# clancylian/retinaface

Measured on NVIDIA H100. Metric: faces/sec (end-to-end detect), higher is better.
Workload: dtype f16

## Files before the change

retinaface_b200/csrc/engine.cu:

```cuda
#include <cmath>

#include "engine_internal.cuh"
#include "calibrate.cuh"
#include "preprocess.cuh"

namespace rf_eng {

std::string &create_error() {
    thread_local std::string text;
    return text;
}

void link_steps(rf_handle h) {
    auto &st = h->steps;
    for (int i = 0; i < (int)st.size(); i++) {
        st[i].deps.clear();
        for (int t : st[i].in) {
            for (int j = i - 1; j >= 0; j--) {
                bool writes = false;
                for (int o : st[j].out) writes |= (o == t);
                if (!writes) continue;
                if (st[j].lane != st[i].lane) {
                    if (std::find(st[i].deps.begin(), st[i].deps.end(), j) == st[i].deps.end()) st[i].deps.push_back(j);
                    st[j].signals = true;
                }
                break;
            }
        }
    }
    for (int l = 1; l < 3; l++) {
        h->lane_last[l] = -1;
        for (int i = 0; i < (int)st.size(); i++) if (st[i].lane == l) h->lane_last[l] = i;
        if (h->lane_last[l] >= 0) st[h->lane_last[l]].signals = true;
    }
}

void place_tensors(rf_handle h, bool keep_all) {
    auto &ts = h->tensors;
    auto &st = h->steps;
    for (int si = 0; si < (int)st.size(); si++) {
        for (int t : st[si].out) { if (ts[t].first < 0) ts[t].first = si; ts[t].last = std::max(ts[t].last, si); }
        for (int t : st[si].in) ts[t].last = std::max(ts[t].last, si);
    }
    for (int k = 0; k < (int)st.size(); k++) {
        if (st[k].lane == 0) continue;
        int join = (int)st.size() - 1;
        for (int j = k + 1; j < (int)st.size() && join == (int)st.size() - 1; j++)
            for (int d : st[j].deps)
                if (st[j].lane != st[k].lane && st[d].lane == st[k].lane && d >= k) { join = j; break; }
        for (int t : st[k].in) ts[t].last = std::max(ts[t].last, join);
        for (int t : st[k].out) ts[t].last = std::max(ts[t].last, join);
    }
    const size_t B = (size_t)h->cfg.max_batch;
    size_t top = 0;
    std::vector<int> order(ts.size());
    for (size_t i = 0; i < ts.size(); i++) order[i] = (int)i;
    std::stable_sort(order.begin(), order.end(), [&](int a, int b) { return ts[a].first < ts[b].first; });
    std::vector<int> placed;
    for (int id : order) {
        size_t sz = (ts[id].bytes_per_img * B + 255) / 256 * 256;
        size_t off = 0;
        if (keep_all) {
            off = top;
        } else {
            bool moved = true;
            while (moved) {
                moved = false;
                for (int p : placed) {
                    bool live_overlap = !(ts[p].last < ts[id].first || ts[id].last < ts[p].first);
                    size_t psz = (ts[p].bytes_per_img * B + 255) / 256 * 256;
                    bool mem_overlap = off < ts[p].offset + psz && ts[p].offset < off + sz;
                    if (live_overlap && mem_overlap) { off = ts[p].offset + psz; moved = true; }
                }
            }
        }
        ts[id].offset = off;
        top = std::max(top, off + sz);
        placed.push_back(id);
    }
    h->arena_bytes = top;
}

void make_plan(rf_handle h, bool init) {
    const rf_config &cfg = h->cfg;
    h->use_tc = cfg.precision == RF_PREC_INT8 || (cfg.precision == RF_PREC_FP16 && !(cfg.flags & RF_FLAG_NO_TENSORCORE));
    if (init && h->use_tc) CK(tc_init());
    if (cfg.precision == RF_PREC_INT8) { if (init) CK(tc_init_i8()); build_plan_i8(h); }
    else if (cfg.precision == RF_PREC_FP32) build_plan<float>(h);
    else if (h->use_tc && !(cfg.flags & RF_FLAG_LEGACY_TC)) { if (init) CK(tile_init()); build_plan_tiles(h); }
    else build_plan<__half>(h);
    link_steps(h);
    place_tensors(h, false);
}

void alloc_post_buffers(PostBuffers &pb, int anchors, int batch, int max_faces) {
    int ap2 = 1;
    while (ap2 < anchors) ap2 <<= 1;
    pb.anchors_per_image = anchors; pb.anchors_pow2 = ap2; pb.max_faces = max_faces; pb.max_batch = batch;
    const size_t B = batch;
    CK(cudaMalloc(&pb.cand_keys, sizeof(unsigned long long) * B * anchors));
    CK(cudaMalloc(&pb.cand_recs, sizeof(rf_det) * B * anchors));
    CK(cudaMalloc(&pb.cand_count, sizeof(int) * B));
    CK(cudaMemset(pb.cand_count, 0, sizeof(int) * B));
    CK(cudaMalloc(&pb.sort_scratch, sizeof(unsigned long long) * B * ap2));
    CK(cudaMalloc(&pb.flag_scratch, B * ap2));
    CK(cudaMalloc(&pb.out_dets, sizeof(rf_det) * B * max_faces));
    CK(cudaMalloc(&pb.out_counts, sizeof(int) * B));
    CK(cudaMalloc(&pb.out_total_kept, sizeof(int) * B));
    CK(cudaMemset(pb.out_counts, 0, sizeof(int) * B));
    CK(cudaMalloc(&pb.tile_done, sizeof(int) * B));
    CK(cudaMemset(pb.tile_done, 0, sizeof(int) * B));
}
void free_post_buffers(PostBuffers &pb) {
    cudaFree(pb.cand_keys); cudaFree(pb.cand_recs); cudaFree(pb.cand_count); cudaFree(pb.sort_scratch); cudaFree(pb.flag_scratch);
    cudaFree(pb.out_dets); cudaFree(pb.out_counts); cudaFree(pb.out_total_kept); cudaFree(pb.tile_done);
    pb = PostBuffers{};
}

void create_ctx(rf_handle h, Ctx &c, bool all) {
    if (all) {
        CK(cudaStreamCreateWithFlags(&c.stream, cudaStreamNonBlocking));
        for (int l = 1; l < 3; l++) CK(cudaStreamCreateWithFlags(&c.lane_stream[l], cudaStreamNonBlocking));
        c.step_event.assign(h->steps.size(), nullptr);
        for (size_t i = 0; i < h->steps.size(); i++)
            if (h->steps[i].signals) CK(cudaEventCreateWithFlags(&c.step_event[i], cudaEventDisableTiming));
        CK(cudaEventCreateWithFlags(&c.fence, cudaEventDisableTiming));
    }
    CK(cudaMalloc(&c.arena, h->arena_bytes));
    if (!all) return;
    CK(cudaMalloc(&c.d_params, sizeof(PostParams)));
    CK(cudaHostAlloc(&c.h_params, sizeof(PostParams) * Ctx::kParamSlots, cudaHostAllocDefault));
    int anchors = 0;
    for (const LevelDesc &lv : h->lv) anchors += 2 * lv.h * lv.w;
    alloc_post_buffers(c.pb, anchors, h->cfg.max_batch, h->cfg.max_faces);
}

void release_ctx(Ctx &c, bool all) {
    if (c.stream) cudaStreamSynchronize(c.stream);
    for (auto &g : c.graphs) cudaGraphExecDestroy(g.second);
    c.graphs.clear();
    cudaFree(c.arena);
    c.arena = nullptr;
    if (!all) return;
    cudaFree(c.d_params); cudaFreeHost(c.h_params);
    free_post_buffers(c.pb);
    for (auto e : c.step_event) if (e) cudaEventDestroy(e);
    for (int l = 1; l < 3; l++) if (c.lane_stream[l]) cudaStreamDestroy(c.lane_stream[l]);
    if (c.fence) cudaEventDestroy(c.fence);
    if (c.stream) cudaStreamDestroy(c.stream);
    c = Ctx{};
}

void run_steps(rf_handle h, const Run &r, bool use_lanes = true) {
    static const bool one_lane = [] { const char *e = getenv("RF_ONE_LANE"); return e && e[0] == '1'; }();
    if (one_lane) use_lanes = false;
    const Ctx &c = r.ctx;
    for (size_t i = 0; i < h->steps.size(); i++) {
        Step &st = h->steps[i];
        cudaStream_t cs = (use_lanes && st.lane) ? c.lane_stream[st.lane] : r.stream;
        if (use_lanes)
            for (int d : st.deps) CK(cudaStreamWaitEvent(cs, c.step_event[d], 0));
        st.launch(Run{c, r.n, cs, r.blobs});
        if (use_lanes && st.signals) CK(cudaEventRecord(c.step_event[i], cs));
    }
    if (use_lanes)
        for (int l = 1; l < 3; l++)
            if (h->lane_last[l] >= 0) CK(cudaStreamWaitEvent(r.stream, c.step_event[h->lane_last[l]], 0));
    if (h->comm.ready) comm_wait_in_graph(h, c, r.n, r.stream);
}

void forward_graph(rf_handle h, Ctx &c, int n) {
    if (h->cfg.flags & RF_FLAG_NO_GRAPH) {
        run_steps(h, Run{c, n, c.stream});
        CK(cudaGetLastError());
        return;
    }
    auto it = c.graphs.find(n);
    if (it == c.graphs.end()) {
        cudaGraph_t g = nullptr;
        CK(cudaStreamBeginCapture(c.stream, cudaStreamCaptureModeThreadLocal));
        run_steps(h, Run{c, n, c.stream});
        cudaError_t e = cudaStreamEndCapture(c.stream, &g);
        if (e != cudaSuccess) throw CudaFail{e, "cudaStreamEndCapture", __FILE__, __LINE__};
        cudaGraphExec_t ge = nullptr;
        e = cudaGraphInstantiate(&ge, g, 0);
        cudaGraphDestroy(g);
        if (e != cudaSuccess) throw CudaFail{e, "cudaGraphInstantiate", __FILE__, __LINE__};
        it = c.graphs.emplace(n, ge).first;
    }
    CK(cudaGraphLaunch(it->second, c.stream));
}

void set_params(rf_handle h, Ctx &c, float thr, float nms, const uint8_t *input = nullptr, unsigned comm_seq = 0) {
    PostParams *slot = c.h_params + (c.param_seq++ % Ctx::kParamSlots);
    slot->score_thr = thr;
    slot->nms_thr = nms;
    slot->input = input ? input : h->d_input;
    slot->comm_seq = comm_seq;
    slot->comm_slot = comm_seq ? comm_seq % (unsigned)h->comm.ring : 0u;
    c.cur_thr = thr;
    c.cur_nms = nms;
    CK(cudaMemcpyAsync(c.d_params, slot, sizeof(PostParams), cudaMemcpyHostToDevice, c.stream));
}

void destroy(rf_handle h) {
    if (!h) return;
    cudaSetDevice(h->device);
    for (Ctx &c : h->ctx) if (c.stream) cudaStreamSynchronize(c.stream);
    comm_release(h);
    jpeg_release(h);
    for (Ctx &c : h->ctx) release_ctx(c, true);
    free_post_buffers(h->pb_merge);
    cudaFree(h->d_weights); cudaFree(h->d_weights_h); cudaFree(h->d_weights_q); cudaFree(h->d_input); cudaFree(h->d_raw);
    for (auto p : h->d_blobs) cudaFree(p);
    h->copy_pool.reset();
    for (auto e : h->raw_ev) if (e) cudaEventDestroy(e);
    cudaFree(h->d_align_images); cudaFreeHost(h->h_align_images); cudaFree(h->d_align_crops); cudaFree(h->d_align_mats);
    cudaFreeHost(h->h_input); cudaFreeHost(h->h_raw); cudaFreeHost(h->h_dets); cudaFreeHost(h->h_counts); cudaFreeHost(h->tile_dbg);
    for (auto &sl : h->slots) {
        cudaFree(sl.d_in); cudaFreeHost(sl.h_in); cudaFreeHost(sl.h_dets); cudaFreeHost(sl.h_counts);
        if (sl.ev_h2d) cudaEventDestroy(sl.ev_h2d);
        if (sl.ev_done) cudaEventDestroy(sl.ev_done);
    }
    if (h->copy_stream) cudaStreamDestroy(h->copy_stream);
    if (h->ev0) cudaEventDestroy(h->ev0);
    if (h->ev1) cudaEventDestroy(h->ev1);
    delete h;
}

int check_n(rf_handle h, int n) {
    if (!h) return RF_ERR_INVALID_ARG;
    if (n < 0) return fail(h, RF_ERR_INVALID_ARG, "negative batch size");
    if (n > h->cfg.max_batch) return fail(h, RF_ERR_CAPACITY, fmt("batch %d exceeds max_batch %d", n, h->cfg.max_batch));
    return RF_OK;
}

}

extern "C" {

int rf_abi_version(void) { return RF_B200_ABI_VERSION; }

const char *rf_build_info(void) {
    return "librf_b200 (RetinaFace mnet25 detect path) built for sm_90a, CUDA " RF_STR(CUDART_VERSION);
}

const char *rf_status_string(int s) {
    switch (s) {
        case RF_OK: return "ok";
        case RF_ERR_INVALID_ARG: return "invalid argument";
        case RF_ERR_IO: return "i/o error";
        case RF_ERR_MODEL: return "model error";
        case RF_ERR_CUDA: return "CUDA error";
        case RF_ERR_NO_DEVICE: return "no usable CUDA device (the library has no CPU path)";
        case RF_ERR_CAPACITY: return "capacity exceeded";
        case RF_ERR_UNSUPPORTED: return "unsupported";
    }
    return "unknown status";
}

const char *rf_last_error(rf_handle h) { return h ? h->err.c_str() : create_error().c_str(); }

int rf_create(const rf_config *cfg, rf_handle *out) {
    if (out) *out = nullptr;
    if (!cfg || !out) return fail(nullptr, RF_ERR_INVALID_ARG, "rf_create: cfg and out must be non-NULL");
    if (!cfg->caffemodel_path) return fail(nullptr, RF_ERR_INVALID_ARG, "rf_create: caffemodel_path is NULL");
    rf_config cfg_local = *cfg;
    NetGraph graph;
    Model model;
    int cache_status = CACHE_NONE;
    {
        std::string err;
        int st = RF_OK;
        if (cfg->network) {
            NetworkConfig nc;
            if (!network_config(cfg->network, nc, err)) return fail(nullptr, RF_ERR_UNSUPPORTED, "rf_create: " + err);
            if (nc.ratios.size() != 1) return fail(nullptr, RF_ERR_UNSUPPORTED, fmt("rf_create: network '%s' uses %zu anchor ratios per scale; the shipped models (and this engine) have 2 anchors per position", cfg->network, nc.ratios.size()));
        }
        if (!load_model(cfg->caffemodel_path, cfg->prototxt_path ? cfg->prototxt_path : "", cfg->cache_path ? cfg->cache_path : "", model, &graph, &cache_status, err, st))
            return fail(nullptr, st, err);
        if (cfg->prototxt_path && cfg_local.net_w == 0 && cfg_local.net_h == 0) { cfg_local.net_h = graph.input_dims[2]; cfg_local.net_w = graph.input_dims[3]; }
    }
    cfg = &cfg_local;
    if (cfg->net_w <= 0 || cfg->net_h <= 0 || cfg->net_w % 32 || cfg->net_h % 32)
        return fail(nullptr, RF_ERR_INVALID_ARG, fmt("rf_create: net size %dx%d must be positive multiples of 32", cfg->net_w, cfg->net_h));
    if (cfg->max_batch <= 0 || cfg->max_batch > 4096) return fail(nullptr, RF_ERR_INVALID_ARG, "rf_create: max_batch must be in [1, 4096]");
    {
        const long long stem_elems = (long long)cfg->max_batch * (cfg->net_h / 2) * (cfg->net_w / 2) * 16;
        const long long merge_rows = (long long)cfg->max_batch * (cfg->net_h / 8);
        if (stem_elems > 0x7fffffffLL || merge_rows >= (1LL << 19) || cfg->net_w / 8 >= (1 << 12))
            return fail(nullptr, RF_ERR_CAPACITY, fmt("rf_create: max_batch %d at %dx%d exceeds the 32-bit activation index range (largest tensor: %lld elements); "
                                                      "use a smaller max_batch", cfg->max_batch, cfg->net_w, cfg->net_h, stem_elems));
    }
    if (cfg->precision != RF_PREC_FP32 && cfg->precision != RF_PREC_FP16 && cfg->precision != RF_PREC_INT8)
        return fail(nullptr, RF_ERR_INVALID_ARG, "rf_create: unknown precision");
    if (cfg->precision == RF_PREC_INT8 && !cfg->int8_table_path)
        return fail(nullptr, RF_ERR_INVALID_ARG, "rf_create: RF_PREC_INT8 needs int8_table_path (the TensorRT calibration cache of this caffemodel)");

    std::unique_ptr<rf_handle_s, void (*)(rf_handle)> H(new rf_handle_s, destroy);
    rf_handle h = H.get();
    h->cfg = *cfg;
    h->caffemodel = cfg->caffemodel_path;
    h->cfg.caffemodel_path = h->caffemodel.c_str();
    if (cfg->int8_table_path) { h->table = cfg->int8_table_path; h->cfg.int8_table_path = h->table.c_str(); }
    if (h->cfg.max_faces <= 0) h->cfg.max_faces = 256;
    if (h->cfg.max_faces > 8192) return fail(nullptr, RF_ERR_INVALID_ARG, "rf_create: max_faces must be <= 8192");
    if (h->cfg.max_image_w <= 0) h->cfg.max_image_w = h->cfg.net_w;
    if (h->cfg.max_image_h <= 0) h->cfg.max_image_h = h->cfg.net_h;
    h->cfg.max_image_w = std::max(h->cfg.max_image_w, h->cfg.net_w);
    h->cfg.max_image_h = std::max(h->cfg.max_image_h, h->cfg.net_h);
    h->device = cfg->device;
    h->elem = cfg->precision == RF_PREC_FP32 ? 4 : (cfg->precision == RF_PREC_FP16 ? 2 : 1);

    {
        std::string err;
        h->model = std::move(model);
        h->cache_status = cache_status;
        h->cfg.prototxt_path = h->cfg.cache_path = h->cfg.network = nullptr;
        if (!h->table.empty() && !read_int8_table(h->table, h->int8_scales, err)) return fail(nullptr, RF_ERR_IO, err);
    }
    int ndev = 0;
    cudaError_t e = cudaGetDeviceCount(&ndev);
    if (e != cudaSuccess || ndev == 0)
        return fail(nullptr, RF_ERR_NO_DEVICE, fmt("no CUDA device (%s); librf_b200 has no CPU path", e == cudaSuccess ? "count 0" : cudaGetErrorString(e)));
    if (cfg->device < 0 || cfg->device >= ndev) return fail(nullptr, RF_ERR_INVALID_ARG, fmt("device %d out of range (%d devices)", cfg->device, ndev));
    try {
        CK(cudaSetDevice(h->device));
        cudaDeviceProp prop;
        CK(cudaGetDeviceProperties(&prop, h->device));
        if (prop.major != 9 || prop.minor != 0)
            return fail(nullptr, RF_ERR_NO_DEVICE, fmt("device %d is sm_%d%d; librf_b200 is built for sm_90a only", h->device, prop.major, prop.minor));
        h->num_sms = prop.multiProcessorCount;
        CK(cudaEventCreate(&h->ev0));
        CK(cudaEventCreate(&h->ev1));
        CK(postproc_init());

        const int Hn = h->cfg.net_h, Wn = h->cfg.net_w, Bm = h->cfg.max_batch;
        const int strides[3] = {32, 16, 8};
        int abase = 0, pbase = 0;
        for (int l = 0; l < 3; l++) {
            LevelDesc &lv = h->lv[l];
            lv.stride = strides[l]; lv.h = Hn / strides[l]; lv.w = Wn / strides[l];
            lv.anchor_base = abase; lv.pix_base = pbase;
            base_anchors_net3(strides[l], lv.base);
            abase += 2 * lv.h * lv.w; pbase += lv.h * lv.w;
        }
        make_plan(h, true);
        CK(cudaMalloc(&h->d_weights, h->wstage.size() * sizeof(float)));
        CK(cudaMemcpy(h->d_weights, h->wstage.data(), h->wstage.size() * sizeof(float), cudaMemcpyHostToDevice));
        if (!h->wstage_h.empty()) {
            CK(cudaMalloc(&h->d_weights_h, h->wstage_h.size() * sizeof(__half)));
            CK(cudaMemcpy(h->d_weights_h, h->wstage_h.data(), h->wstage_h.size() * sizeof(__half), cudaMemcpyHostToDevice));
        }
        if (!h->wstage_q.empty()) {
            CK(cudaMalloc(&h->d_weights_q, h->wstage_q.size()));
            CK(cudaMemcpy(h->d_weights_q, h->wstage_q.data(), h->wstage_q.size(), cudaMemcpyHostToDevice));
        }
        const size_t in_bytes = (size_t)Bm * Hn * Wn * 3;
        CK(cudaMalloc(&h->d_input, in_bytes));
        CK(cudaHostAlloc(&h->h_input, in_bytes, cudaHostAllocDefault));
        h->raw_bytes = ((size_t)h->cfg.max_image_w * h->cfg.max_image_h * 3 + 255) / 256 * 256;
        h->raw_slots = (int)std::max<size_t>(1, std::min<size_t>((size_t)Bm, ((size_t)2 << 30) / h->raw_bytes));
        CK(cudaMalloc(&h->d_raw, h->raw_bytes * h->raw_slots));
        CK(cudaHostAlloc(&h->h_raw, 2 * h->raw_bytes, cudaHostAllocDefault));
        for (auto &e : h->raw_ev) CK(cudaEventCreateWithFlags(&e, cudaEventDisableTiming));
        CK(cudaHostAlloc(&h->h_dets, sizeof(rf_det) * (size_t)Bm * h->cfg.max_faces, cudaHostAllocDefault));
        CK(cudaHostAlloc(&h->h_counts, sizeof(int) * 2 * Bm, cudaHostAllocDefault));
        CK(cudaHostAlloc(&h->tile_dbg, 64, cudaHostAllocMapped));
        memset(h->tile_dbg, 0, 64);
        CK(cudaHostGetDevicePointer(&h->tile_dbg_dev, h->tile_dbg, 0));
        h->ctx.resize(h->cfg.streams <= 0 ? RF_MAX_STREAMS : std::min(h->cfg.streams, RF_MAX_STREAMS));
        for (Ctx &c : h->ctx) create_ctx(h, c, true);
        for (int l = 0; l < 3; l++) {
            const int ch[3] = {4, 8, 20};
            for (int k = 0; k < 3; k++) h->blob_elems[3 * l + k] = (size_t)ch[k] * h->lv[l].h * h->lv[l].w;
        }
        CK(cudaDeviceSynchronize());
    } catch (const CudaFail &f) {
        return fail_cuda(nullptr, f);
    } catch (const PlanFail &f) {
        return fail(nullptr, f.status, "rf_create: " + f.msg);
    }
    *out = H.release();
    return RF_OK;
}

void rf_destroy(rf_handle h) { destroy(h); }

// ... 850 lines not shown
```

retinaface_b200/csrc/engine_internal.cuh:

```cuda
#pragma once
#include <algorithm>
#include <cstdarg>
#include <cstdio>
#include <cstring>
#include <functional>
#include <map>
#include <memory>
#include <string>
#include <type_traits>
#include <vector>

#include "align.cuh"
#include "common.cuh"
#include "host_copy.h"
#include "model.h"
#include "postproc.cuh"
#include "preprocess.cuh"

using namespace rf;

#define RF_STR2(x) #x
#define RF_STR(x) RF_STR2(x)

namespace rf_eng {

constexpr int RF_NUM_SMS = 132;

struct TileChain;
std::string &create_error();

struct CudaFail { cudaError_t e; const char *what; const char *file; int line; };
struct PlanFail { int status; std::string msg; };
#define CK(call)                                                        \
    do {                                                                \
        cudaError_t _e = (call);                                        \
        if (_e != cudaSuccess) throw CudaFail{_e, #call, __FILE__, __LINE__}; \
    } while (0)

inline std::string fmt(const char *f, ...) {
    char buf[1024];
    va_list ap;
    va_start(ap, f);
    vsnprintf(buf, sizeof buf, f, ap);
    va_end(ap);
    return buf;
}

struct TensorInfo {
    std::string name;
    int h = 0, w = 0, c = 0;
    size_t bytes_per_img = 0;
    int first = -1, last = -1;
    size_t offset = 0;
};

struct Ctx {
    static constexpr int kParamSlots = 1024;
    cudaStream_t stream = nullptr, lane_stream[3] = {nullptr, nullptr, nullptr};
    std::vector<cudaEvent_t> step_event;
    unsigned char *arena = nullptr;
    PostBuffers pb{};
    PostParams *d_params = nullptr, *h_params = nullptr;
    unsigned param_seq = 0;
    float cur_thr = 0.5f, cur_nms = 0.4f;
    std::map<int, cudaGraphExec_t> graphs;
    cudaEvent_t fence = nullptr;
};

struct Run {
    const Ctx &ctx;
    int n;
    cudaStream_t stream;
    float *const *blobs = nullptr;
    bool single = false;
};

struct Step {
    std::string name;
    std::vector<int> in, out;
    std::function<void(const Run &)> launch;
    double flops_per_img = 0, bytes_per_img = 0;
    int lane = 0;
    std::vector<int> deps;
    bool signals = false;
};

}
using namespace rf_eng;

namespace rf_eng {
struct Comm {
    int rank = 0, world = 1, ring = 0;
    bool ready = false;
    unsigned char *window = nullptr;
    size_t bytes = 0;
    unsigned char *peer[RF_COMM_MAX_WORLD] = {nullptr};
    bool opened[RF_COMM_MAX_WORLD] = {false};
    unsigned seq = 0;
    unsigned *d_err = nullptr, *h_err = nullptr;
    unsigned char blob[128] = {0};
    struct Slot { rf_det *h_dets = nullptr; int *h_counts = nullptr; } slots[RF_PIPELINE_DEPTH];
};
}

struct rf_handle_s {
    rf_config cfg{};
    rf_eng::Comm comm;
    std::string caffemodel, table;
    std::string err;
    Model model;
    std::map<std::string, float> int8_scales;
    int device = 0;
    int num_sms = RF_NUM_SMS;
    int elem = 4;
    cudaEvent_t ev0 = nullptr, ev1 = nullptr;

    std::vector<TensorInfo> tensors;
    std::map<std::string, int> tensor_by_name;
    std::vector<Step> steps;
    int head_step = -1, nms_step = -1;
    std::vector<std::shared_ptr<TileChain>> chains;
    unsigned tile_mask = 0;
    int lane_last[3] = {-1, -1, -1};
    int cache_status = 0;
    int tile_expected = 0;
    std::vector<float> tile_bias_tmp;
    unsigned *tile_dbg = nullptr, *tile_dbg_dev = nullptr;
    size_t arena_bytes = 0;

    std::vector<float> wstage;
    float *d_weights = nullptr;
    std::vector<__half> wstage_h;
    __half *d_weights_h = nullptr;
    std::vector<int8_t> wstage_q;
    int8_t *d_weights_q = nullptr;
    bool use_tc = false;

    uint8_t *d_input = nullptr;
    uint8_t *h_input = nullptr;
    PostBuffers pb_merge{};
    uint8_t *d_raw = nullptr;
    uint8_t *h_raw = nullptr;
    size_t raw_bytes = 0;
    int raw_slots = 1;
    cudaEvent_t raw_ev[2] = {nullptr, nullptr};
    unsigned raw_seq = 0;
    std::unique_ptr<HostCopyPool> copy_pool;
    AlignImage *d_align_images = nullptr, *h_align_images = nullptr;
    void *d_align_crops = nullptr;
    size_t align_crops_bytes = 0;
    double *d_align_mats = nullptr;
    LevelDesc lv[3];
    HeadWeights hw[3];
    int feat_tensor[3] = {-1, -1, -1};
    float *d_blobs[9] = {nullptr};
    size_t blob_elems[9] = {0};
    rf_det *h_dets = nullptr;
    int *h_counts = nullptr;
    struct Slot {
        uint8_t *d_in = nullptr, *h_in = nullptr;
        rf_det *h_dets = nullptr;
        int *h_counts = nullptr;
        cudaEvent_t ev_h2d = nullptr, ev_done = nullptr;
        int n = 0;
        bool busy = false, gather = false;
    } slots[RF_PIPELINE_DEPTH];
    cudaStream_t copy_stream = nullptr;
    unsigned submit_seq = 0, collect_seq = 0;
    std::vector<Ctx> ctx;
    unsigned next_dev_ctx = 0;
    cudaStream_t last_stream = nullptr;
    void *jpeg = nullptr;
};

namespace rf_eng {
inline int fail(rf_handle h, int code, const std::string &msg) {
    if (h) h->err = msg; else create_error() = msg;
    return code;
}
inline int fail_cuda(rf_handle h, const CudaFail &f) {
    std::string extra;
    if (h && h->tile_dbg && h->tile_dbg[0])
        extra = fmt(" [tile chain: CTA %u timed out waiting at tile_chain.cuh:%u]", h->tile_dbg[0] >> 20, h->tile_dbg[0] & 0xfffffu);
    return fail(h, RF_ERR_CUDA, fmt("%s failed: %s (%s:%d)%s", f.what, cudaGetErrorString(f.e), f.file, f.line, extra.c_str()));
}

struct Builder {
    rf_handle h;
    int H, W;
    size_t add_weights(const std::vector<float> &v) {
        size_t off = h->wstage.size();
        h->wstage.insert(h->wstage.end(), v.begin(), v.end());
        while (h->wstage.size() % 4) h->wstage.push_back(0.f);
        return off;
    }
    size_t add_weights_h(const std::vector<__half> &v) {
        size_t off = h->wstage_h.size();
        h->wstage_h.insert(h->wstage_h.end(), v.begin(), v.end());
        while (h->wstage_h.size() % 64) h->wstage_h.push_back(__float2half(0.f));
        return off;
    }
    size_t add_weights_q(const std::vector<int8_t> &v) {
        size_t off = h->wstage_q.size();
        h->wstage_q.insert(h->wstage_q.end(), v.begin(), v.end());
        while (h->wstage_q.size() % 128) h->wstage_q.push_back(0);
        return off;
    }
    int tensor(const std::string &name, int hh, int ww, int c) {
        TensorInfo t;
        t.name = name; t.h = hh; t.w = ww; t.c = c;
        t.bytes_per_img = (size_t)hh * ww * c * h->elem;
        h->tensors.push_back(t);
        h->tensor_by_name[name] = (int)h->tensors.size() - 1;
        return (int)h->tensors.size() - 1;
    }
    void step(Step s) { h->steps.push_back(std::move(s)); }
};

constexpr int TC_SMEM_LIMIT = 200 * 1024;
struct DwGeom { int rows, nsplit, Rmax; };
template <typename T>
void build_plan(rf_handle h);
cudaError_t tc_init();
std::vector<__half> make_stem_blob(const std::vector<float> &w0, const std::vector<float> &b0, const std::vector<float> &wd,
                                   const std::vector<float> &bd, const std::vector<float> &wp, const std::vector<float> &bp);
int plan_stem_tc(Builder &B);
int plan_pair_legacy(Builder &B, int i, int tin, int ih, int iw);
void plan_conv_legacy(Builder &B, const std::string &sname, std::vector<const FoldedConv *> cs, int tin, int ih, int iw, int t0, int ld0,
                      int off0, int n0, int relu0, int t1, int ld1, int off1, int relu1, int lane = 0, int tup = -1, int up_which = 0);
int plan_fpn_merge_h2(Builder &B, const std::string &name, int tlat, int tup, int fh, int fw, int which);
template <typename T>
void plan_heads_and_nms(Builder &B, bool with_heads, bool with_nms);
std::vector<__half> pack_tc_weights(const std::vector<const FoldedConv *> &cs, std::vector<float> &bias, int &Kpad, int nsplit = 1);
void build_plan_tiles(rf_handle h);
cudaError_t tile_init();
std::string describe_chains(rf_handle h);
void comm_release(rf_handle h);
void comm_wait_in_graph(rf_handle h, const Ctx &c, int n, cudaStream_t s);
int jpeg_info(rf_handle h, const uint8_t *data, size_t len, int *w, int *hgt);
int jpeg_decode(rf_handle h, const uint8_t *const *data, const size_t *len, int n, uint8_t *const *dst, const int *w, const int *hgt, cudaStream_t s);
void jpeg_release(rf_handle h);
const char *jpeg_backend(rf_handle h);
void build_plan_i8(rf_handle h);
cudaError_t tc_init_i8();

}
```

retinaface_b200/csrc/plan_fp.cu:

```cuda
#include "engine_internal.cuh"
#include "kernels_simt.cuh"
#include "stem_tc.cuh"
#include "tc_conv.cuh"
#include "tc_dwpw2d.cuh"

namespace rf_eng {

#define CK_L(...) CK(launch_k(__VA_ARGS__))

std::vector<float> pack_gemm(const std::vector<const FoldedConv *> &cs, std::vector<float> &bias) {
    const int cin = cs[0]->cin, k = cs[0]->k;
    int N = 0;
    for (auto c : cs) N += c->cout;
    std::vector<float> w((size_t)k * k * cin * N);
    bias.assign(N, 0.f);
    int n0 = 0;
    for (auto c : cs) {
        for (int o = 0; o < c->cout; o++) {
            bias[n0 + o] = c->b[o];
            for (int ci = 0; ci < cin; ci++)
                for (int t = 0; t < k * k; t++)
                    w[((size_t)t * cin + ci) * N + n0 + o] = c->w[((size_t)o * cin + ci) * k * k + t];
        }
        n0 += c->cout;
    }
    return w;
}

template <typename T>
void launch_gemm(const T *in, int ldin, int cin, const float *wk, const float *bias, int N, int ks, OutSplit<T> outs,
                 int n, int H, int W, cudaStream_t s) {
    long M = (long)n * H * W;
    int bn = (N % 64 == 0) ? 64 : (N % 32 == 0 ? 32 : 16);
    dim3 grid((unsigned)((M + 63) / 64), (N + bn - 1) / bn);
#define RF_GEMM(BN_, KS_) CK_L(k_conv_gemm<T, BN_, KS_>, grid, dim3(256), 0, s, in, ldin, cin, wk, bias, N, outs, n, H, W)
    if (ks == 1) { if (bn == 64) RF_GEMM(64, 1); else if (bn == 32) RF_GEMM(32, 1); else RF_GEMM(16, 1); }
    else { if (bn == 64) RF_GEMM(64, 3); else if (bn == 32) RF_GEMM(32, 3); else RF_GEMM(16, 3); }
#undef RF_GEMM
}

std::vector<__half> pack_tc_weights(const std::vector<const FoldedConv *> &cs, std::vector<float> &bias, int &Kpad, int nsplit) {
    const int cin = cs[0]->cin, k = cs[0]->k;
    int N = 0;
    for (auto c : cs) N += c->cout;
    const int K = k * k * cin;
    Kpad = (K + 15) / 16 * 16;
    const int Ns = N / nsplit;
    std::vector<__half> img((size_t)Kpad * N, __float2half(0.f));
    bias.assign(N, 0.f);
    int n0 = 0;
    for (auto c : cs) {
        for (int o = 0; o < c->cout; o++) {
            const int n = n0 + o, sl = n / Ns, nl = n % Ns;
            bias[n] = c->b[o];
            for (int ci = 0; ci < cin; ci++)
                for (int t = 0; t < k * k; t++) {
                    const int kk = t * cin + ci;
                    img[(size_t)sl * Kpad * Ns + ((size_t)(kk / 8) * Ns + nl) * 8 + (kk % 8)] =
                        __float2half(c->w[((size_t)o * cin + ci) * k * k + t]);
                }
        }
        n0 += c->cout;
    }
    return img;
}

void launch_tc_conv(const TcConvArgs &a_in, cudaStream_t s) {
    TcConvArgs a = a_in;
    a.mul_Wp = fast_div_mul((uint32_t)a.Wp); a.mul_Hp = fast_div_mul((uint32_t)a.Hp); a.mul_H = fast_div_mul((uint32_t)a.H);
    const long P = (long)a.nimg * a.Hp * a.Wp;
    const unsigned grid = (unsigned)((P + 127) / 128);
    const size_t smem = tc_conv_smem_bytes(a);
    switch (tc_n_bucket(a.N)) {
        case 32: if (a.up) CK_L(k_tc_conv_staged<32, true>, dim3(grid), dim3(TC_THREADS), smem, s, a); else CK_L(k_tc_conv_staged<32, false>, dim3(grid), dim3(TC_THREADS), smem, s, a); break;
        case 64: if (a.up) CK_L(k_tc_conv_staged<64, true>, dim3(grid), dim3(TC_THREADS), smem, s, a); else CK_L(k_tc_conv_staged<64, false>, dim3(grid), dim3(TC_THREADS), smem, s, a); break;
        case 128: if (a.up) CK_L(k_tc_conv_staged<128, true>, dim3(grid), dim3(TC_THREADS), smem, s, a); else CK_L(k_tc_conv_staged<128, false>, dim3(grid), dim3(TC_THREADS), smem, s, a); break;
        default: if (a.up) CK_L(k_tc_conv_staged<256, true>, dim3(grid), dim3(TC_THREADS), smem, s, a); else CK_L(k_tc_conv_staged<256, false>, dim3(grid), dim3(TC_THREADS), smem, s, a); break;
    }
}
void launch_tc_dwpw(const TcDwArgs &a_in, int nsplit, cudaStream_t s) {
    TcDwArgs a = a_in;
    a.mul_Wp = fast_div_mul((uint32_t)a.Wp); a.mul_Hp = fast_div_mul((uint32_t)a.Hp);
    a.mul_OW = fast_div_mul((uint32_t)a.OW); a.mul_OH = fast_div_mul((uint32_t)a.OH);
    const long M = (long)a.nimg * a.OH * a.OW;
    dim3 grid((unsigned)((M + a.rows - 1) / a.rows), nsplit);
    const size_t smem = tc_dw_smem_bytes(a);
    switch (tc_n_bucket(a.N)) {
        case 32: CK_L(k_tc_dwpw_staged<32>, grid, dim3(TC_THREADS), smem, s, a); break;
        case 64: CK_L(k_tc_dwpw_staged<64>, grid, dim3(TC_THREADS), smem, s, a); break;
        case 128: CK_L(k_tc_dwpw_staged<128>, grid, dim3(TC_THREADS), smem, s, a); break;
        default: CK_L(k_tc_dwpw_staged<256>, grid, dim3(TC_THREADS), smem, s, a); break;
    }
}
void launch_tc_dwpw_2d(const TcDw2dArgs &a, cudaStream_t s) {
    const dim3 grid((unsigned)(a.tiles_x * a.tiles_y * a.nimg));
    const size_t smem = tc_dw2d_smem_bytes(a);
    switch (tc_n_bucket(a.N)) {
        case 32: CK_L(k_tc_dwpw_2d<32>, grid, dim3(TC_THREADS), smem, s, a); break;
        case 64: CK_L(k_tc_dwpw_2d<64>, grid, dim3(TC_THREADS), smem, s, a); break;
        case 128: CK_L(k_tc_dwpw_2d<128>, grid, dim3(TC_THREADS), smem, s, a); break;
        default: CK_L(k_tc_dwpw_2d<256>, grid, dim3(TC_THREADS), smem, s, a); break;
    }
}

cudaError_t tc_init() {
    cudaError_t e;
#define RF_TC_ATTR(K_) if ((e = cudaFuncSetAttribute(K_, cudaFuncAttributeMaxDynamicSharedMemorySize, TC_SMEM_LIMIT))) return e
    RF_TC_ATTR((k_tc_conv_staged<32, false>)); RF_TC_ATTR((k_tc_conv_staged<64, false>)); RF_TC_ATTR((k_tc_conv_staged<128, false>)); RF_TC_ATTR((k_tc_conv_staged<256, false>));
    RF_TC_ATTR((k_tc_conv_staged<32, true>)); RF_TC_ATTR((k_tc_conv_staged<64, true>)); RF_TC_ATTR((k_tc_conv_staged<128, true>)); RF_TC_ATTR((k_tc_conv_staged<256, true>));
    RF_TC_ATTR(k_tc_dwpw_staged<32>); RF_TC_ATTR(k_tc_dwpw_staged<64>); RF_TC_ATTR(k_tc_dwpw_staged<128>); RF_TC_ATTR(k_tc_dwpw_staged<256>);
    RF_TC_ATTR(k_tc_dwpw_2d<32>); RF_TC_ATTR(k_tc_dwpw_2d<64>); RF_TC_ATTR(k_tc_dwpw_2d<128>); RF_TC_ATTR(k_tc_dwpw_2d<256>);
#undef RF_TC_ATTR
    return cudaSuccess;
}

DwGeom dw_geometry(int C, int N, int IH, int IW, int S) {
    const int OH = IH / S, OW = IW / S, Wp = IW + 2, Hp = IH + 1, Kpad = (C + 15) / 16 * 16;
    auto centre = [&](long m) { long ox = m % OW, oy = (m / OW) % OH, b = m / ((long)OW * OH); return (b * Hp + oy * S) * Wp + ox * S + 1; };
    for (int rows : {128, 64}) {
        if (rows == 128 && OH * OW <= 28 * 28) continue;
        for (int nsplit : {1, 2, 4}) {
            if ((N / nsplit) % 16) continue;
            long g = rows, t = (long)OH * OW;
            while (t) { long u = g % t; g = t; t = u; }
            const long M = ((long)rows / g + 1) * OH * OW;
            int R = 0;
            for (long m0 = 0; m0 < M; m0 += rows) {
                long ml = std::min(m0 + rows, M) - 1;
                R = std::max(R, (int)(centre(ml) - centre(m0) + 2 * (Wp + 1) + 1));
            }
            R |= 1;
            TcDwArgs a{};
            a.C = C; a.Rmax = R; a.Kpad = Kpad; a.N = N / nsplit; a.rows = rows;
            if (R <= TC_MAX_R && tc_dw_smem_bytes(a) <= (size_t)TC_SMEM_LIMIT) return {rows, nsplit, R};
        }
    }
    return {0, 0, 0};
}

std::vector<__half> make_stem_blob(const std::vector<float> &w0, const std::vector<float> &b0, const std::vector<float> &wd,
                                          const std::vector<float> &bd, const std::vector<float> &wp, const std::vector<float> &bp) {
    std::vector<__half> b0img(2 * 4 * 16 * 8, __float2half(0.f)), b1img(2 * 16 * 8, __float2half(0.f));
    for (int k = 0; k < 27; k++)
        for (int o = 0; o < 8; o++) {
            const float wv = w0[k * 8 + o];
            const __half hi = __float2half(wv);
            b0img[((k / 8) * 16 + o) * 8 + (k % 8)] = hi;
            b0img[((4 + k / 8) * 16 + o) * 8 + (k % 8)] = __float2half(wv - __half2float(hi));
        }
    for (int c = 0; c < 8; c++)
        for (int o = 0; o < 16; o++) b1img[(0 * 16 + o) * 8 + c] = __float2half(wp[c * 16 + o]);
    std::vector<__half> blob(STEM_CONST_BYTES / 2, __float2half(0.f));
    memcpy(blob.data(), b0img.data(), STEM_B0_BYTES);
    memcpy(reinterpret_cast<unsigned char *>(blob.data()) + STEM_B0_BYTES, b1img.data(), STEM_B1_BYTES);
    std::vector<float> fl;
    fl.insert(fl.end(), b0.begin(), b0.begin() + 8);
    fl.insert(fl.end(), wd.begin(), wd.begin() + 72);
    fl.insert(fl.end(), bd.begin(), bd.begin() + 8);
    fl.insert(fl.end(), bp.begin(), bp.begin() + 16);
    fl.insert(fl.end(), wp.begin(), wp.begin() + 128);
    memcpy(reinterpret_cast<unsigned char *>(blob.data()) + STEM_B0_BYTES + STEM_B1_BYTES, fl.data(), STEM_F_FLOATS * 4);
    return blob;
}


int plan_pair_legacy(Builder &B, int i, int tin, int ih, int iw) {
    rf_handle h = B.h;
    const Model &m = h->model;
    auto T_ = [h](const Run &r, int id) { return reinterpret_cast<__half *>(r.ctx.arena + h->tensors[id].offset); };
    auto Wd = [h](size_t off) { return h->d_weights + off; };
    const double es = h->elem;
    const FoldedConv &dw = m.conv("mobilenet0_conv" + std::to_string(i) + "_fwd");
    const FoldedConv &pw = m.conv("mobilenet0_conv" + std::to_string(i + 1) + "_fwd");
    const int C = dw.cout, S = dw.stride;
    std::vector<float> wd(9 * C);
    for (int c = 0; c < C; c++)
        for (int t = 0; t < 9; t++) wd[t * C + c] = dw.w[(size_t)c * 9 + t];
    size_t owd = B.add_weights(wd), obd = B.add_weights(dw.b);
    const int oh = ih / S, ow_ = iw / S;
    const int N = pw.cout;
    const DwGeom geo = dw_geometry(C, N, ih, iw, S);
    if (geo.rows == 0) throw PlanFail{RF_ERR_UNSUPPORTED, fmt("layer mobilenet0_conv%d (%dx%d, %d channels) does not fit shared memory", i, iw, ih, C)};
    std::vector<float> bias;
    int Kpad = 0;
    std::vector<__half> img = pack_tc_weights({&pw}, bias, Kpad, geo.nsplit);
    size_t oimg = B.add_weights_h(img), obp = B.add_weights(bias);
    int tpw = B.tensor("mobilenet0_relu" + std::to_string(i + 1) + "_fwd", oh, ow_, N);
    Step s;
    s.name = fmt("tc_dw%d+pw%d_s%d_%dto%d", i, i + 1, S, C, N);
    s.in = {tin}; s.out = {tpw};
    s.flops_per_img = 2.0 * oh * ow_ * C * 9 + 2.0 * oh * ow_ * C * N;
    s.bytes_per_img = ((double)ih * iw * C + (double)oh * ow_ * N) * es;
    const bool tiles2d = oh * ow_ > 56 * 56 && C >= 16 && C <= 64 && geo.nsplit == 1 && !(h->cfg.flags & RF_FLAG_DW_1D);
    if (tiles2d) s.name = fmt("tc2d_dw%d+pw%d_s%d_%dto%d", i, i + 1, S, C, N);
    s.launch = [=](const Run &r) {
        if (tiles2d) {
            TcDw2dArgs a{};
            a.in = T_(r, tin); a.C = C; a.nimg = r.n; a.IH = ih; a.IW = iw; a.OH = oh; a.OW = ow_; a.S = S; a.N = N;
            a.TH = 8;
            const int t16 = (ow_ + 15) / 16, t14 = (ow_ + 13) / 14;
            a.TW = t14 < t16 ? 14 : 16;
            tc_dw2d_finish(a);
            a.wimg = h->d_weights_h + oimg; a.bias = Wd(obp); a.dw_w = Wd(owd); a.dw_b = Wd(obd); a.out = T_(r, tpw);
            launch_tc_dwpw_2d(a, r.stream);
            return;
        }
        TcDwArgs a{};
        a.in = T_(r, tin); a.C = C; a.nimg = r.n; a.IH = ih; a.IW = iw; a.OH = oh; a.OW = ow_; a.S = S;
        a.N = N / geo.nsplit; a.Ntotal = N; a.Kpad = Kpad; a.rows = geo.rows; a.Wp = iw + 2; a.Hp = ih + 1; a.Rmax = geo.Rmax;
        a.wimg = h->d_weights_h + oimg; a.bias = Wd(obp); a.dw_w = Wd(owd); a.dw_b = Wd(obd); a.out = T_(r, tpw);
        launch_tc_dwpw(a, geo.nsplit, r.stream);
    };
    B.step(std::move(s));
    return tpw;
}

void plan_conv_legacy(Builder &B, const std::string &sname, std::vector<const FoldedConv *> cs, int tin, int ih, int iw, int t0, int ld0,
                      int off0, int n0, int relu0, int t1, int ld1, int off1, int relu1, int lane, int tup, int up_which) {
    rf_handle h = B.h;
    const Model &m = h->model;
    auto T_ = [h](const Run &r, int id) { return reinterpret_cast<__half *>(r.ctx.arena + h->tensors[id].offset); };
    auto Wd = [h](size_t off) { return h->d_weights + off; };
    const double es = h->elem;
    std::vector<float> bias;
    int Kpad = 0;
    std::vector<__half> img = pack_tc_weights(cs, bias, Kpad);
    size_t oimg = B.add_weights_h(img), ob = B.add_weights(bias);
    const int N = (int)bias.size(), cin = cs[0]->cin, ks = cs[0]->k;
    size_t oup = tup >= 0 ? B.add_weights(m.up_w[up_which]) : 0;
    if (cin & (cin - 1)) throw PlanFail{RF_ERR_UNSUPPORTED, fmt("convolution %s: %d input channels (the tensor-core kernels index by shifts: powers of two only)", sname.c_str(), cin)};
    TcConvArgs probe{};
    probe.Cin = cin; probe.taps = ks * ks; probe.N = N; probe.R = (ks == 3 ? 128 + 2 * (iw + 3) : 128) | 1;
    if (tup >= 0) { probe.up = reinterpret_cast<const __half *>(1); probe.Cmax = (((probe.R / (iw + 2) + 2) / 2 + 3) * (iw / 2)) | 1; }
    if (tc_conv_smem_bytes(probe) > (size_t)TC_SMEM_LIMIT || probe.R > TC_MAX_R)
        throw PlanFail{RF_ERR_UNSUPPORTED, fmt("convolution %s (%dx%d map) does not fit shared memory", sname.c_str(), iw, ih)};
    Step s;
    s.name = "tc_" + sname;
    s.lane = lane;
    s.in = {tin};
    if (tup >= 0) s.in.push_back(tup);
    s.out = {t0};
    if (t1 >= 0) s.out.push_back(t1);
    s.flops_per_img = 2.0 * ih * iw * cin * ks * ks * N + (tup >= 0 ? 2.0 * ih * iw * cin * 4 : 0.0);
    s.bytes_per_img = ((double)ih * iw * cin + (double)ih * iw * N + (tup >= 0 ? (double)(ih / 2) * (iw / 2) * cin : 0.0)) * es;
    s.launch = [=](const Run &r) {
        TcConvArgs a{};
        a.in = T_(r, tin); a.Cin = cin; a.nimg = r.n; a.H = ih; a.W = iw; a.taps = ks * ks; a.N = N;
        a.Wp = ks == 3 ? iw + 2 : iw; a.Hp = ks == 3 ? ih + 1 : ih;
        a.R = (ks == 3 ? 128 + 2 * (iw + 3) : 128) | 1;
        a.wimg = h->d_weights_h + oimg; a.bias = Wd(ob);
        a.out = TcOut{T_(r, t0) + off0, ld0, n0, relu0, t1 >= 0 ? T_(r, t1) + off1 : nullptr, ld1, relu1};
        if (tup >= 0) { a.up = T_(r, tup); a.up_w = Wd(oup); a.Cmax = (((a.R / a.Wp + 2) / 2 + 3) * (iw / 2)) | 1; }
        launch_tc_conv(a, r.stream);
    };
    B.step(std::move(s));
}

int plan_fpn_merge_h2(Builder &B, const std::string &name, int tlat, int tup, int fh, int fw, int which) {
    rf_handle h = B.h;
    const Model &m = h->model;
    auto T_ = [h](const Run &r, int id) { return reinterpret_cast<__half *>(r.ctx.arena + h->tensors[id].offset); };
    const double es = h->elem;
    std::vector<__half> uwh(16 * 64);
    for (int c = 0; c < 64; c++)
        for (int t = 0; t < 16; t++) uwh[t * 64 + c] = __float2half(m.up_w[which][c * 16 + t]);
    size_t ouw = B.add_weights_h(uwh);
    int plus = B.tensor(name, fh, fw, 64);
    Step s;
    s.name = "fpn_merge" + name + "_upsample+add_h2";
    s.in = {tlat, tup}; s.out = {plus};
    s.flops_per_img = 2.0 * fh * fw * 64 * 4;
    s.bytes_per_img = ((double)fh * fw * 64 * 2 + (double)(fh / 2) * (fw / 2) * 64) * es;
    s.launch = [=](const Run &r) {
        CK(launch_k(k_fpn_merge_h2, dim3((unsigned)((fw * 8 + 127) / 128), (unsigned)fh, (unsigned)r.n), dim3(128), 0, r.stream, (const __half *)T_(r, tlat), (const __half *)T_(r, tup),
                    (__half *)T_(r, plus), (const __half *)(h->d_weights_h + ouw), r.n, fh, fw, 64));
    };
    B.step(std::move(s));
    return plus;
}

template <typename T>
void plan_heads_and_nms(Builder &B, bool with_heads, bool with_nms) {
    rf_handle h = B.h;
    const Model &m = h->model;
    auto T_ = [h](const Run &r, int id) { return reinterpret_cast<T *>(r.ctx.arena + h->tensors[id].offset); };
    auto Wd = [h](size_t off) { return h->d_weights + off; };
    const double es = h->elem;
    const int H = h->cfg.net_h, W = h->cfg.net_w;
    const int h32 = H / 32, w32 = W / 32, h16 = H / 16, w16 = W / 16, h8 = H / 8, w8 = W / 8;
    if (with_heads) {
        size_t hw_off[3], hb_off[3];
        const int strides[3] = {32, 16, 8};
        for (int l = 0; l < 3; l++) {
            std::string st = "_stride" + std::to_string(strides[l]);
            const FoldedConv *cs[3] = {&m.conv("face_rpn_cls_score" + st), &m.conv("face_rpn_bbox_pred" + st),
                                       &m.conv("face_rpn_landmark_pred" + st)};
            std::vector<float> w(32 * 64), b(32);
            int r = 0;
            for (auto c : cs)
                for (int o = 0; o < c->cout; o++, r++) {
                    b[r] = c->b[o];
                    for (int ci = 0; ci < 64; ci++) w[r * 64 + ci] = c->w[(size_t)o * 64 + ci];
                }
            hw_off[l] = B.add_weights(w);
            hb_off[l] = B.add_weights(b);
        }
        Step s;
        s.name = "heads_1x1+softmax+decode_all_levels";
        s.in = {h->feat_tensor[0], h->feat_tensor[1], h->feat_tensor[2]};
        double px = (double)h32 * w32 + (double)h16 * w16 + (double)h8 * w8;
        s.flops_per_img = 2.0 * px * 64 * 4;
        s.bytes_per_img = px * 64 * es;
        int f0 = h->feat_tensor[0], f1 = h->feat_tensor[1], f2 = h->feat_tensor[2];
        size_t w0 = hw_off[0], w1 = hw_off[1], w2 = hw_off[2], b0 = hb_off[0], b1 = hb_off[1], b2 = hb_off[2];
        s.launch = [=](const Run &r) {
            const T *feat[3] = {T_(r, f0), T_(r, f1), T_(r, f2)};
            HeadWeights hws[3] = {{Wd(w0), Wd(b0), 1.f}, {Wd(w1), Wd(b1), 1.f}, {Wd(w2), Wd(b2), 1.f}};
            launch_head_decode<T>(feat, hws, h->lv, r.n, W, H, r.ctx.d_params, r.ctx.pb, r.blobs, r.stream, with_nms);
        };
        if (with_nms) s.name = "heads_1x1+softmax+decode+nms_all_levels";
        h->head_step = (int)h->steps.size();
        B.step(std::move(s));
        if (with_nms) return;
    }
    if (with_nms) {
        Step s;
        s.name = "sort+nms";
        s.in = {h->feat_tensor[0], h->feat_tensor[1], h->feat_tensor[2]};
        s.flops_per_img = 0;
        s.bytes_per_img = 0;
        s.launch = [=](const Run &r) { launch_nms(r.n, r.ctx.d_params, r.ctx.pb, r.stream); };
        h->nms_step = (int)h->steps.size();
        B.step(std::move(s));
    }
}
template void plan_heads_and_nms<float>(Builder &, bool, bool);
template void plan_heads_and_nms<__half>(Builder &, bool, bool);

int plan_stem_tc(Builder &B) {
    rf_handle h = B.h;
    const Model &m = h->model;
    const int H = h->cfg.net_h, W = h->cfg.net_w;
    auto T_ = [h](const Run &r, int id) { return reinterpret_cast<__half *>(r.ctx.arena + h->tensors[id].offset); };
    auto Wd = [h](size_t off) { return h->d_weights + off; };
    const double es = h->elem;
    const int cur_h = H / 2, cur_w = W / 2;
    const FoldedConv &c0 = m.conv("mobilenet0_conv0_fwd"), &dw = m.conv("mobilenet0_conv1_fwd"), &pw = m.conv("mobilenet0_conv2_fwd");
    std::vector<float> w0(27 * 8), wd(72), wp(128);
    for (int o = 0; o < 8; o++)
        for (int cb = 0; cb < 3; cb++)
            for (int t = 0; t < 9; t++) w0[(t * 3 + cb) * 8 + o] = c0.w[((size_t)o * 3 + (2 - cb)) * 9 + t];
    for (int c = 0; c < 8; c++)
        for (int t = 0; t < 9; t++) wd[t * 8 + c] = dw.w[(size_t)c * 9 + t];
    for (int o = 0; o < 16; o++)
        for (int c = 0; c < 8; c++) wp[c * 16 + o] = pw.w[(size_t)o * 8 + c];
    size_t ow0 = B.add_weights(w0), ob0 = B.add_weights(c0.b), owd = B.add_weights(wd), obd = B.add_weights(dw.b),
           owp = B.add_weights(wp), obp = B.add_weights(pw.b);
    std::vector<__half> blob = make_stem_blob(w0, c0.b, wd, dw.b, wp, pw.b);
    size_t oblob = B.add_weights_h(blob);
    const bool simt_stem = (h->cfg.flags & (RF_FLAG_SIMT_STEM | RF_FLAG_NO_TENSORCORE)) != 0;
    int out = B.tensor("mobilenet0_relu2_fwd", cur_h, cur_w, 16);
    Step s;
    s.name = simt_stem ? "stem_conv0+dw1+pw2_u8_to_16ch" : "tc_stem_conv0+dw1+pw2_u8_to_16ch";
    s.out = {out};
    s.flops_per_img = 2.0 * cur_h * cur_w * (8 * 27 + 8 * 9 + 8 * 16);
    s.bytes_per_img = (double)H * W * 3 + (double)cur_h * cur_w * 16 * es;
    s.launch = [=](const Run &r) {
        const int tiles = ((H / 2 + 15) / 16) * ((W / 2 + 15) / 16);
        if (simt_stem) {
            StemWeights sw{Wd(ow0), Wd(ob0), Wd(owd), Wd(obd), Wd(owp), Wd(obp)};
            CK(launch_k(k_stem<__half>, dim3((unsigned)(tiles * r.n)), dim3(256), 0, r.stream, (const PostParams *)r.ctx.d_params, (__half *)T_(r, out), sw, r.n, H, W, 1.0f));
        } else {
            StemTcArgs a{reinterpret_cast<const unsigned char *>(h->d_weights_h + oblob)};
            CK(launch_k(k_stem_tc<__half>, dim3((unsigned)((W / 2 + 15) / 16), (unsigned)((H / 2 + 15) / 16), (unsigned)r.n), dim3(256), 0, r.stream, (const PostParams *)r.ctx.d_params, (__half *)T_(r, out), a, r.n, H, W, 1.0f));
        }
    };
    B.step(std::move(s));
    return out;
}

template <typename T>
void build_plan(rf_handle h) {
    Builder B{h, h->cfg.net_h, h->cfg.net_w};
    const Model &m = h->model;
    const int H = h->cfg.net_h, W = h->cfg.net_w;
    auto T_ = [h](const Run &r, int id) { return reinterpret_cast<T *>(r.ctx.arena + h->tensors[id].offset); };
    auto Wd = [h](size_t off) { return h->d_weights + off; };
    const double es = h->elem;

    int first_pair = 1;
    int cur_h = H / 2, cur_w = W / 2, cur_c = 8;
    int cur = -1;
    bool stem_done = false;
    if constexpr (std::is_same<T, __half>::value) {
        if (h->use_tc) {
            cur = plan_stem_tc(B);
            cur_c = 16;
            first_pair = 3;
            stem_done = true;
        }
    }
    if (!stem_done) {
    cur = B.tensor("mobilenet0_relu0_fwd", cur_h, cur_w, 8);
    {
        const FoldedConv &c = m.conv("mobilenet0_conv0_fwd");
        std::vector<float> wk(27 * 8);
        for (int o = 0; o < 8; o++)
            for (int cb = 0; cb < 3; cb++)
                for (int t = 0; t < 9; t++) wk[(t * 3 + cb) * 8 + o] = c.w[((size_t)o * 3 + (2 - cb)) * 9 + t];
        size_t ow = B.add_weights(wk), ob = B.add_weights(c.b);
        int out = cur;
        Step s;
        s.name = "conv0_u8_3x3s2_bn_relu";
        s.out = {out};
        s.flops_per_img = 2.0 * cur_h * cur_w * 8 * 27;
        s.bytes_per_img = (double)H * W * 3 + (double)cur_h * cur_w * 8 * es;
        s.launch = [=](const Run &r) {
            long total = (long)r.n * (H / 2) * (W / 2);
            CK_L(k_conv0<T>, dim3((unsigned)((total + 255) / 256)), dim3(256), 0, r.stream, (const PostParams *)r.ctx.d_params, T_(r, out), Wd(ow), Wd(ob), r.n, H, W);
        };
        B.step(std::move(s));
    }
    }
    int c1 = -1, c2 = -1, c3 = -1;
    for (int i = first_pair; i <= 26; i += 2) {
        const FoldedConv &dw = m.conv("mobilenet0_conv" + std::to_string(i) + "_fwd");
        const FoldedConv &pw = m.conv("mobilenet0_conv" + std::to_string(i + 1) + "_fwd");
        const int C = dw.cout, S = dw.stride;
        std::vector<float> wd(9 * C);
        for (int c = 0; c < C; c++)
            for (int t = 0; t < 9; t++) wd[t * C + c] = dw.w[(size_t)c * 9 + t];
        size_t owd = B.add_weights(wd), obd = B.add_weights(dw.b);
        const int ih = cur_h, iw = cur_w, oh = cur_h / S, ow_ = cur_w / S;
        int tin = cur;
        if constexpr (std::is_same<T, __half>::value) {
            if (h->use_tc) {
                cur = plan_pair_legacy(B, i, tin, ih, iw);
                cur_h = oh; cur_w = ow_; cur_c = pw.cout;
                if (i + 1 == 10) c1 = cur;
                if (i + 1 == 22) c2 = cur;
                if (i + 1 == 26) c3 = cur;
                continue;
            }
        }
        int tdw = B.tensor("mobilenet0_relu" + std::to_string(i) + "_fwd", oh, ow_, C);
        {
            Step s;
            s.name = fmt("dw%d_3x3s%d_c%d", i, S, C);
            s.in = {tin}; s.out = {tdw};
            s.flops_per_img = 2.0 * oh * ow_ * C * 9;
            s.bytes_per_img = ((double)ih * iw * C + (double)oh * ow_ * C) * es;
            s.launch = [=](const Run &r) {
                long total = (long)r.n * oh * ow_ * (C / 8);
                unsigned g = (unsigned)((total + 255) / 256);
                if (S == 1) CK_L(k_dw3x3<T, 1>, dim3(g), dim3(256), 0, r.stream, (const T *)T_(r, tin), T_(r, tdw), Wd(owd), Wd(obd), r.n, ih, iw, C);
                else CK_L(k_dw3x3<T, 2>, dim3(g), dim3(256), 0, r.stream, (const T *)T_(r, tin), T_(r, tdw), Wd(owd), Wd(obd), r.n, ih, iw, C);
            };
            B.step(std::move(s));
        }
        std::vector<float> bias;
        std::vector<float> wk = pack_gemm({&pw}, bias);
        size_t owp = B.add_weights(wk), obp = B.add_weights(bias);
        const int N = pw.cout;
        int tpw = B.tensor("mobilenet0_relu" + std::to_string(i + 1) + "_fwd", oh, ow_, N);
        {
            Step s;
            s.name = fmt("pw%d_1x1_%dto%d", i + 1, C, N);
            s.in = {tdw}; s.out = {tpw};
            s.flops_per_img = 2.0 * oh * ow_ * C * N;
            s.bytes_per_img = ((double)oh * ow_ * C + (double)oh * ow_ * N) * es;
            s.launch = [=](const Run &r) {
                OutSplit<T> o{T_(r, tpw), N, N, 1, nullptr, 0, 0};
                launch_gemm<T>(T_(r, tdw), C, C, Wd(owp), Wd(obp), N, 1, o, r.n, oh, ow_, r.stream);
            };
            B.step(std::move(s));
        }
        cur = tpw; cur_h = oh; cur_w = ow_; cur_c = N;
        if (i + 1 == 10) c1 = cur;
        if (i + 1 == 22) c2 = cur;
        if (i + 1 == 26) c3 = cur;
    }
    (void)cur_c;

    auto conv_step = [&](const std::string &sname, std::vector<const FoldedConv *> cs, int tin, int ih, int iw,
                         int t0, int ld0, int off0, int n0, int relu0, int t1, int ld1, int off1, int relu1, int lane = 0,
                         int tup = -1, int up_which = 0) {
        if constexpr (std::is_same<T, __half>::value) {
            if (h->use_tc) {
                plan_conv_legacy(B, sname, cs, tin, ih, iw, t0, ld0, off0, n0, relu0, t1, ld1, off1, relu1, lane, tup, up_which);
                return;
            }
        }
        std::vector<float> bias;
        std::vector<float> wk = pack_gemm(cs, bias);
        size_t ow = B.add_weights(wk), ob = B.add_weights(bias);
        const int N = (int)bias.size(), cin = cs[0]->cin, ks = cs[0]->k;
        const int ldin = h->tensors[tin].c;
        Step s;
        s.name = sname;
        s.lane = lane;
        s.in = {tin};
        s.out = {t0};
        if (t1 >= 0) s.out.push_back(t1);
        s.flops_per_img = 2.0 * ih * iw * cin * ks * ks * N;
        s.bytes_per_img = ((double)ih * iw * cin + (double)ih * iw * N) * es;
        s.launch = [=](const Run &r) {
            OutSplit<T> o{T_(r, t0) + off0, ld0, n0, relu0, t1 >= 0 ? T_(r, t1) + off1 : nullptr, ld1, relu1};
            launch_gemm<T>(T_(r, tin), ldin, cin, Wd(ow), Wd(ob), N, ks, o, r.n, ih, iw, r.stream);
        };
        B.step(std::move(s));
    };
    auto ssh = [&](const std::string &lvname, int tin, int fh, int fw, int level, int lane) {
        const std::string p = "rf_" + lvname + "_det";
        int cat = B.tensor(p + "_concat_relu", fh, fw, 64);
        int ctx1 = B.tensor(p + "_context_conv1_relu", fh, fw, 16);
        int ctx31 = B.tensor(p + "_context_conv3_1_relu", fh, fw, 16);
        conv_step("ssh_" + lvname + "_conv1+ctx1_3x3_64to48", {&m.conv(p + "_conv1"), &m.conv(p + "_context_conv1")}, tin, fh,
                  fw, cat, 64, 0, 32, 1, ctx1, 16, 0, 1, lane);
        conv_step("ssh_" + lvname + "_ctx2+ctx3_1_3x3_16to32", {&m.conv(p + "_context_conv2"), &m.conv(p + "_context_conv3_1")},
                  ctx1, fh, fw, cat, 64, 32, 16, 1, ctx31, 16, 0, 1, lane);
        conv_step("ssh_" + lvname + "_ctx3_2_3x3_16to16", {&m.conv(p + "_context_conv3_2")}, ctx31, fh, fw, cat, 64, 48, 16, 1,
                  -1, 0, 0, 0, lane);
        h->feat_tensor[level] = cat;
    };
    auto upadd = [&](const std::string &name, int tlat, int tup, int fh, int fw, int which) {
        size_t ow = B.add_weights(m.up_w[which]);
        int out = B.tensor(name, fh, fw, 64);
        Step s;
        s.name = "upsample_add" + name;
        s.in = {tlat, tup}; s.out = {out};
        s.flops_per_img = 2.0 * fh * fw * 64 * 4;
        s.bytes_per_img = ((double)fh * fw * 64 * 2 + (double)(fh / 2) * (fw / 2) * 64) * es;
        s.launch = [=](const Run &r) {
            long total = (long)r.n * fh * fw * 8;
            CK_L(k_upsample_add<T>, dim3((unsigned)((total + 255) / 256)), dim3(256), 0, r.stream, (const T *)T_(r, tlat), (const T *)T_(r, tup), T_(r, out), Wd(ow), r.n,
                     fh, fw, 64, fh / 2, fw / 2);
        };
        B.step(std::move(s));
        return out;
    };
    const int h32 = H / 32, w32 = W / 32, h16 = H / 16, w16 = W / 16, h8 = H / 8, w8 = W / 8;
    const bool lanes = h->use_tc;
    auto move_last_step_after_producer = [&](int tensor_id) {
        int pos = 0;
        for (int i = (int)h->steps.size() - 2; i >= 0 && !pos; i--)
            for (int t : h->steps[i].out) if (t == tensor_id) { pos = i + 1; break; }
        Step st = std::move(h->steps.back());
        h->steps.pop_back();
        h->steps.insert(h->steps.begin() + pos, std::move(st));
    };
    int lat3 = B.tensor("rf_c3_lateral_relu", h32, w32, 64);
    int lat2 = B.tensor("rf_c2_lateral_relu", h16, w16, 64);
    int lat1 = B.tensor("rf_c1_red_conv_relu", h8, w8, 64);
    conv_step("c1_red_1x1_64to64", {&m.conv("rf_c1_red_conv")}, c1, h8, w8, lat1, 64, 0, 64, 1, -1, 0, 0, 0, lanes ? 1 : 0);
    if (lanes) move_last_step_after_producer(c1);
    conv_step("c2_lateral_1x1_128to64", {&m.conv("rf_c2_lateral")}, c2, h16, w16, lat2, 64, 0, 64, 1, -1, 0, 0, 0, lanes ? 2 : 0);
    if (lanes) move_last_step_after_producer(c2);
    conv_step("c3_lateral_1x1_256to64", {&m.conv("rf_c3_lateral")}, c3, h32, w32, lat3, 64, 0, 64, 1, -1, 0, 0, 0);
    ssh("c3", lat3, h32, w32, 0, lanes ? 1 : 0);
    int aggr2 = B.tensor("rf_c2_aggr_relu", h16, w16, 64);
    if (h->use_tc) {
        conv_step("c2_upsample+add+aggr_3x3_64to64", {&m.conv("rf_c2_aggr")}, lat2, h16, w16, aggr2, 64, 0, 64, 1, -1, 0, 0, 0, 0, lat3, 0);
    } else {
        int plus0 = upadd("_plus0", lat2, lat3, h16, w16, 0);
        conv_step("c2_aggr_3x3_64to64", {&m.conv("rf_c2_aggr")}, plus0, h16, w16, aggr2, 64, 0, 64, 1, -1, 0, 0, 0);
    }
    ssh("c2", aggr2, h16, w16, 1, lanes ? 2 : 0);
    int aggr1 = B.tensor("rf_c1_aggr_relu", h8, w8, 64);
    const long c1_tiles = ((long)h->cfg.max_batch * (h8 + 1) * (w8 + 2) + 127) / 128;
    if (h->use_tc && c1_tiles <= h->num_sms) {
        conv_step("c1_upsample+add+aggr_3x3_64to64", {&m.conv("rf_c1_aggr")}, lat1, h8, w8, aggr1, 64, 0, 64, 1, -1, 0, 0, 0, 0, aggr2, 1);
    } else if (h->use_tc) {
        if constexpr (std::is_same<T, __half>::value) {
            int plus1 = plan_fpn_merge_h2(B, "_plus1", lat1, aggr2, h8, w8, 1);
            conv_step("c1_aggr_3x3_64to64", {&m.conv("rf_c1_aggr")}, plus1, h8, w8, aggr1, 64, 0, 64, 1, -1, 0, 0, 0);
        }
    } else {
        int plus1 = upadd("_plus1", lat1, aggr2, h8, w8, 1);
        conv_step("c1_aggr_3x3_64to64", {&m.conv("rf_c1_aggr")}, plus1, h8, w8, aggr1, 64, 0, 64, 1, -1, 0, 0, 0);
    }
    ssh("c1", aggr1, h8, w8, 2, 0);

    plan_heads_and_nms<T>(B, true, true);
}

template void build_plan<float>(rf_handle h);
template void build_plan<__half>(rf_handle h);

}
```

retinaface_b200/csrc/plan_i8.cu:

```cuda
#include "engine_internal.cuh"
#include "kernels_simt.cuh"
#include "stem_tc.cuh"
#include "tc_conv_i8.cuh"
#include "tc_dwpw2d_i8.cuh"

namespace rf_eng {

struct QWeights { std::vector<int8_t> img; std::vector<float> mult, bq; };

QWeights pack_tc_weights_i8(const std::vector<const FoldedConv *> &cs, float s_in, const std::vector<float> &s_out, int groups, int nsplit) {
    const int cin = cs[0]->cin, k = cs[0]->k, taps = k * k;
    int N = 0;
    for (auto c : cs) N += c->cout;
    const int Ns = N / nsplit;
    QWeights q;
    q.img.assign((size_t)taps * groups * 16 * N, 0);
    q.mult.resize(N); q.bq.resize(N);
    int n0 = 0;
    for (auto c : cs) {
        const size_t per = (size_t)cin * taps;
        for (int o = 0; o < c->cout; o++) {
            const int n = n0 + o, sl = n / Ns, nl = n % Ns;
            float mx = 0.f;
            for (size_t i = 0; i < per; i++) mx = std::max(mx, std::fabs(c->w[o * per + i]));
            const float sw = mx > 0.f ? mx / 127.0f : 1.0f;
            q.mult[n] = (float)((double)s_in * (double)sw / (double)s_out[n]);
            q.bq[n] = (float)((double)c->b[o] / (double)s_out[n]);
            for (int ci = 0; ci < cin; ci++)
                for (int t = 0; t < taps; t++) {
                    double v = std::nearbyint((double)c->w[((size_t)o * cin + ci) * taps + t] / (double)sw);
                    v = std::max(-127.0, std::min(127.0, v));
                    const int g = t * groups + ci / 16;
                    q.img[(size_t)sl * taps * groups * 16 * Ns + ((size_t)g * Ns + nl) * 16 + (ci % 16)] = (int8_t)v;
                }
        }
        n0 += c->cout;
    }
    return q;
}

void launch_tc_conv_i8(const TcConvArgsI8 &a_in, cudaStream_t s) {
    TcConvArgsI8 a = a_in;
    a.mul_Wp = fast_div_mul((uint32_t)a.Wp); a.mul_Hp = fast_div_mul((uint32_t)a.Hp); a.mul_H = fast_div_mul((uint32_t)a.H);
    const long P = (long)a.nimg * a.Hp * a.Wp;
    const dim3 grid((unsigned)((P + 127) / 128));
    const size_t smem = tc_conv_i8_smem_bytes(a);
#define RF_I8C(NT_) if (a.up) launch_k(k_tc_conv_staged_i8<NT_, true>, grid, dim3(TC_THREADS), smem, s, a); else launch_k(k_tc_conv_staged_i8<NT_, false>, grid, dim3(TC_THREADS), smem, s, a)
    switch (tc_n_bucket(a.N)) {
        case 32: RF_I8C(32); break;
        case 64: RF_I8C(64); break;
        case 128: RF_I8C(128); break;
        default: RF_I8C(256); break;
    }
#undef RF_I8C
}
void launch_tc_dwpw_2d_i8(const TcDw2dArgsI8 &a, cudaStream_t s) {
    const dim3 grid((unsigned)a.tiles_x, (unsigned)a.tiles_y, (unsigned)a.nimg);
    const size_t smem = tc_dw2d_i8_smem_bytes(a);
    switch (tc_n_bucket(a.N)) {
        case 32: launch_k(k_tc_dwpw_2d_i8<32>, grid, dim3(TC_THREADS), smem, s, a); break;
        case 64: launch_k(k_tc_dwpw_2d_i8<64>, grid, dim3(TC_THREADS), smem, s, a); break;
        case 128: launch_k(k_tc_dwpw_2d_i8<128>, grid, dim3(TC_THREADS), smem, s, a); break;
        default: launch_k(k_tc_dwpw_2d_i8<256>, grid, dim3(TC_THREADS), smem, s, a); break;
    }
}

void launch_tc_dwpw_i8(const TcDwArgsI8 &a_in, int nsplit, cudaStream_t s) {
    TcDwArgsI8 a = a_in;
    a.mul_Wp = fast_div_mul((uint32_t)a.Wp); a.mul_Hp = fast_div_mul((uint32_t)a.Hp);
    a.mul_OW = fast_div_mul((uint32_t)a.OW); a.mul_OH = fast_div_mul((uint32_t)a.OH);
    const long M = (long)a.nimg * a.OH * a.OW;
    const dim3 grid((unsigned)((M + a.rows - 1) / a.rows), nsplit);
    const size_t smem = tc_dw_i8_smem_bytes(a);
    switch (tc_n_bucket(a.N)) {
        case 32: if (a.C >= 64) launch_k(k_tc_dwpw_staged_i8<32, true>, grid, dim3(TC_THREADS), smem, s, a); else launch_k(k_tc_dwpw_staged_i8<32, false>, grid, dim3(TC_THREADS), smem, s, a); break;
        case 64: if (a.C >= 64) launch_k(k_tc_dwpw_staged_i8<64, true>, grid, dim3(TC_THREADS), smem, s, a); else launch_k(k_tc_dwpw_staged_i8<64, false>, grid, dim3(TC_THREADS), smem, s, a); break;
        case 128: if (a.C >= 64) launch_k(k_tc_dwpw_staged_i8<128, true>, grid, dim3(TC_THREADS), smem, s, a); else launch_k(k_tc_dwpw_staged_i8<128, false>, grid, dim3(TC_THREADS), smem, s, a); break;
        default: if (a.C >= 64) launch_k(k_tc_dwpw_staged_i8<256, true>, grid, dim3(TC_THREADS), smem, s, a); else launch_k(k_tc_dwpw_staged_i8<256, false>, grid, dim3(TC_THREADS), smem, s, a); break;
    }
}
cudaError_t tc_init_i8() {
    cudaError_t e;
#define RF_TC_ATTR(K_) if ((e = cudaFuncSetAttribute(K_, cudaFuncAttributeMaxDynamicSharedMemorySize, TC_SMEM_LIMIT))) return e
    RF_TC_ATTR((k_tc_conv_staged_i8<32, false>)); RF_TC_ATTR((k_tc_conv_staged_i8<64, false>)); RF_TC_ATTR((k_tc_conv_staged_i8<128, false>)); RF_TC_ATTR((k_tc_conv_staged_i8<256, false>));
    RF_TC_ATTR((k_tc_conv_staged_i8<32, true>)); RF_TC_ATTR((k_tc_conv_staged_i8<64, true>)); RF_TC_ATTR((k_tc_conv_staged_i8<128, true>)); RF_TC_ATTR((k_tc_conv_staged_i8<256, true>));
    RF_TC_ATTR((k_tc_dwpw_staged_i8<32, true>)); RF_TC_ATTR((k_tc_dwpw_staged_i8<64, true>)); RF_TC_ATTR((k_tc_dwpw_staged_i8<128, true>)); RF_TC_ATTR((k_tc_dwpw_staged_i8<256, true>));
    RF_TC_ATTR((k_tc_dwpw_staged_i8<32, false>)); RF_TC_ATTR((k_tc_dwpw_staged_i8<64, false>)); RF_TC_ATTR((k_tc_dwpw_staged_i8<128, false>)); RF_TC_ATTR((k_tc_dwpw_staged_i8<256, false>));
    RF_TC_ATTR(k_tc_dwpw_2d_i8<32>); RF_TC_ATTR(k_tc_dwpw_2d_i8<64>); RF_TC_ATTR(k_tc_dwpw_2d_i8<128>); RF_TC_ATTR(k_tc_dwpw_2d_i8<256>);
#undef RF_TC_ATTR
    return cudaSuccess;
}

DwGeom dw_geometry_i8(int C, int N, int IH, int IW, int S) {
    const int OH = IH / S, OW = IW / S, Wp = IW + 2, Hp = IH + 1, Kpad = (C + 31) / 32 * 32;
    auto centre = [&](long m) { long ox = m % OW, oy = (m / OW) % OH, b = m / ((long)OW * OH); return (b * Hp + oy * S) * Wp + ox * S + 1; };
    for (int rows : {128, 64}) {
        if (rows == 128 && OH * OW <= 28 * 28) continue;
        for (int nsplit : {1, 2, 4}) {
            if ((N / nsplit) % 16) continue;
            long g = rows, t = (long)OH * OW;
            while (t) { long u = g % t; g = t; t = u; }
            const long M = ((long)rows / g + 1) * OH * OW;
            int R = 0;
            for (long m0 = 0; m0 < M; m0 += rows) {
                long ml = std::min(m0 + rows, M) - 1;
                R = std::max(R, (int)(centre(ml) - centre(m0) + 2 * (Wp + 1) + 1));
            }
            R |= 1;
            TcDwArgsI8 a{};
            a.C = C; a.Rmax = R; a.Kpad = Kpad; a.N = N / nsplit; a.rows = rows;
            if (R <= TC_MAX_R && tc_dw_i8_smem_bytes(a) <= (size_t)TC_SMEM_LIMIT) return {rows, nsplit, R};
        }
    }
    return {0, 0, 0};
}

void build_plan_i8(rf_handle h) {
    Builder B{h, h->cfg.net_h, h->cfg.net_w};
    const Model &m = h->model;
    const int H = h->cfg.net_h, W = h->cfg.net_w;
    auto Q_ = [h](const Run &r, int id) { return reinterpret_cast<int8_t *>(r.ctx.arena + h->tensors[id].offset); };
    auto Wd = [h](size_t off) { return h->d_weights + off; };
    auto scale_of = [h](const std::string &name) -> float {
        auto it = h->int8_scales.find(name);
        if (it == h->int8_scales.end()) throw PlanFail{RF_ERR_MODEL, "INT8 calibration table lacks the scale of tensor '" + name + "'"};
        return it->second;
    };
    auto tscale = [&](int id) { return scale_of(h->tensors[id].name); };

    int cur_h = H / 2, cur_w = W / 2;
    int cur = B.tensor("mobilenet0_relu2_fwd", cur_h, cur_w, 16);
    {
        const FoldedConv &c0 = m.conv("mobilenet0_conv0_fwd"), &dw = m.conv("mobilenet0_conv1_fwd"), &pw = m.conv("mobilenet0_conv2_fwd");
        std::vector<float> w0(27 * 8), wd(72), wp(128);
        for (int o = 0; o < 8; o++)
            for (int cb = 0; cb < 3; cb++)
                for (int t = 0; t < 9; t++) w0[(t * 3 + cb) * 8 + o] = c0.w[((size_t)o * 3 + (2 - cb)) * 9 + t];
        for (int c = 0; c < 8; c++)
            for (int t = 0; t < 9; t++) wd[t * 8 + c] = dw.w[(size_t)c * 9 + t];
        for (int o = 0; o < 16; o++)
            for (int c = 0; c < 8; c++) wp[c * 16 + o] = pw.w[(size_t)o * 8 + c];
        size_t ow0 = B.add_weights(w0), ob0 = B.add_weights(c0.b), owd = B.add_weights(wd), obd = B.add_weights(dw.b),
               owp = B.add_weights(wp), obp = B.add_weights(pw.b);
        const float inv = 1.0f / tscale(cur);
        int out = cur;
        Step s;
        s.name = "stem_conv0+dw1+pw2_u8_to_16ch_i8";
        s.out = {out};
        s.flops_per_img = 2.0 * cur_h * cur_w * (8 * 27 + 8 * 9 + 8 * 16);
        s.bytes_per_img = (double)H * W * 3 + (double)cur_h * cur_w * 16;
        const bool simt_stem = (h->cfg.flags & (RF_FLAG_SIMT_STEM | RF_FLAG_NO_TENSORCORE)) != 0;
        size_t oblob = B.add_weights_h(make_stem_blob(w0, c0.b, wd, dw.b, wp, pw.b));
        if (!simt_stem) s.name = "tc_stem_conv0+dw1+pw2_u8_to_16ch_i8";
        s.launch = [=](const Run &r) {
            if (simt_stem) {
                StemWeights sw{Wd(ow0), Wd(ob0), Wd(owd), Wd(obd), Wd(owp), Wd(obp)};
                const int tiles = ((H / 2 + 15) / 16) * ((W / 2 + 15) / 16);
                launch_k(k_stem<int8_t>, dim3((unsigned)(tiles * r.n)), dim3(256), 0, r.stream, (const PostParams *)r.ctx.d_params, Q_(r, out), sw, r.n, H, W, inv);
            } else {
                StemTcArgs a{reinterpret_cast<const unsigned char *>(h->d_weights_h + oblob)};
                launch_k(k_stem_tc<int8_t>, dim3((unsigned)((W / 2 + 15) / 16), (unsigned)((H / 2 + 15) / 16), (unsigned)r.n), dim3(256), 0, r.stream,
                         (const PostParams *)r.ctx.d_params, Q_(r, out), a, r.n, H, W, inv);
            }
        };
        B.step(std::move(s));
    }
    int c1 = -1, c2 = -1, c3 = -1;
    for (int i = 3; i <= 26; i += 2) {
        const FoldedConv &dw = m.conv("mobilenet0_conv" + std::to_string(i) + "_fwd");
        const FoldedConv &pw = m.conv("mobilenet0_conv" + std::to_string(i + 1) + "_fwd");
        const int C = dw.cout, S = dw.stride, N = pw.cout;
        const int ih = cur_h, iw = cur_w, oh = cur_h / S, ow_ = cur_w / S;
        const float s_in = tscale(cur), s_mid = scale_of("mobilenet0_relu" + std::to_string(i) + "_fwd");
        std::vector<float> wd(9 * C);
        for (int c = 0; c < C; c++)
            for (int t = 0; t < 9; t++) wd[t * C + c] = dw.w[(size_t)c * 9 + t] * s_in;
        size_t owd = B.add_weights(wd), obd = B.add_weights(dw.b);
        const DwGeom geo = dw_geometry_i8(C, N, ih, iw, S);
        if (geo.rows == 0) throw PlanFail{RF_ERR_UNSUPPORTED, fmt("INT8 layer mobilenet0_conv%d (%dx%d, %d channels) does not fit shared memory", i, iw, ih, C)};
        int tin = cur;
        int tpw = B.tensor("mobilenet0_relu" + std::to_string(i + 1) + "_fwd", oh, ow_, N);
        const int Kpad = (C + 31) / 32 * 32;
        std::vector<float> s_out(N, tscale(tpw));
        QWeights q = pack_tc_weights_i8({&pw}, s_mid, s_out, Kpad / 16, geo.nsplit);
        size_t oimg = B.add_weights_q(q.img), omul = B.add_weights(q.mult), obq = B.add_weights(q.bq);
        const float inv_mid = 1.0f / s_mid;
        Step s;
        s.name = fmt("i8_dw%d+pw%d_s%d_%dto%d", i, i + 1, S, C, N);
        s.in = {tin}; s.out = {tpw};
        s.flops_per_img = 2.0 * oh * ow_ * C * 9 + 2.0 * oh * ow_ * C * N;
        s.bytes_per_img = (double)ih * iw * C + (double)oh * ow_ * N;
        const bool tiles2d = oh * ow_ > 56 * 56 && C >= 16 && C <= 64 && geo.nsplit == 1 && !(h->cfg.flags & RF_FLAG_DW_1D);
        if (tiles2d) s.name = fmt("i8_2d_dw%d+pw%d_s%d_%dto%d", i, i + 1, S, C, N);
        s.launch = [=](const Run &r) {
            if (tiles2d) {
                TcDw2dArgsI8 a{};
                a.in = Q_(r, tin); a.C = C; a.nimg = r.n; a.IH = ih; a.IW = iw; a.OH = oh; a.OW = ow_; a.S = S; a.N = N; a.Kpad = Kpad;
                a.TH = 8;
                a.TW = (ow_ + 13) / 14 < (ow_ + 15) / 16 ? 14 : 16;
                tc_dw2d_i8_finish(a);
                a.wimg = h->d_weights_q + oimg; a.mult = Wd(omul); a.bq = Wd(obq); a.dw_w = Wd(owd); a.dw_b = Wd(obd); a.inv_mid = inv_mid;
                a.out = Q_(r, tpw);
                launch_tc_dwpw_2d_i8(a, r.stream);
                return;
            }
            TcDwArgsI8 a{};
            a.in = Q_(r, tin); a.C = C; a.nimg = r.n; a.IH = ih; a.IW = iw; a.OH = oh; a.OW = ow_; a.S = S;
            a.N = N / geo.nsplit; a.Ntotal = N; a.Kpad = Kpad; a.rows = geo.rows; a.Wp = iw + 2; a.Hp = ih + 1; a.Rmax = geo.Rmax;
            a.wimg = h->d_weights_q + oimg; a.mult = Wd(omul); a.bq = Wd(obq); a.dw_w = Wd(owd); a.dw_b = Wd(obd); a.inv_mid = inv_mid;
            a.out = Q_(r, tpw);
            launch_tc_dwpw_i8(a, geo.nsplit, r.stream);
        };
        B.step(std::move(s));
        cur = tpw; cur_h = oh; cur_w = ow_;
        if (i + 1 == 10) c1 = cur;
        if (i + 1 == 22) c2 = cur;
        if (i + 1 == 26) c3 = cur;
    }
    auto conv_step = [&](const std::string &sname, std::vector<const FoldedConv *> cs, int tin, int ih, int iw, int t0, int ld0, int off0,
                         int n0, int relu0, int t1, int ld1, int off1, int relu1, int lane, int tup, int up_which, int tlat_for_up) {
        (void)tlat_for_up;
        const int cin = cs[0]->cin, ks = cs[0]->k;
        int N = 0;
        for (auto c : cs) N += c->cout;
        std::vector<float> s_out(N);
        for (int n = 0; n < N; n++) s_out[n] = n < n0 ? tscale(t0) : tscale(t1);
        const float s_in = tup >= 0 ? scale_of(up_which == 0 ? "_plus0" : "_plus1") : tscale(tin);
        QWeights q = pack_tc_weights_i8(cs, s_in, s_out, tc_i8_gs(cin), 1);
        size_t oimg = B.add_weights_q(q.img), omul = B.add_weights(q.mult), obq = B.add_weights(q.bq);
        size_t oup = 0;
        float lat_mul = 0.f;
        if (tup >= 0) {
            std::vector<float> wq(16 * cin);
            const float s_up = tscale(tup);
            for (int c = 0; c < cin; c++)
                for (int t = 0; t < 16; t++) wq[t * cin + c] = (float)((double)m.up_w[up_which][c * 16 + t] * (double)s_up / (double)s_in);
            oup = B.add_weights(wq);
            lat_mul = (float)((double)tscale(tin) / (double)s_in);
        }
        Step s;
        s.name = "i8_" + sname;
        s.lane = lane;
        s.in = {tin};
        if (tup >= 0) s.in.push_back(tup);
        s.out = {t0};
        if (t1 >= 0) s.out.push_back(t1);
        s.flops_per_img = 2.0 * ih * iw * cin * ks * ks * N;
        s.bytes_per_img = (double)ih * iw * cin + (double)ih * iw * N + (tup >= 0 ? (double)(ih / 2) * (iw / 2) * cin : 0.0);
        s.launch = [=](const Run &r) {
            TcConvArgsI8 a{};
            a.in = Q_(r, tin); a.Cin = cin; a.nimg = r.n; a.H = ih; a.W = iw; a.taps = ks * ks; a.N = N;
            a.Wp = ks == 3 ? iw + 2 : iw; a.Hp = ks == 3 ? ih + 1 : ih;
            a.R = (ks == 3 ? 128 + 2 * (iw + 3) : 128) | 1;
            a.wimg = h->d_weights_q + oimg; a.mult = Wd(omul); a.bq = Wd(obq);
            a.out = TcOutI8{Q_(r, t0) + off0, ld0, n0, relu0, t1 >= 0 ? Q_(r, t1) + off1 : nullptr, ld1, relu1};
            if (tup >= 0) { a.up = Q_(r, tup); a.up_wq = Wd(oup); a.lat_mul = lat_mul; a.Cmax = (((a.R / a.Wp + 2) / 2 + 3) * (iw / 2)) | 1; }
            launch_tc_conv_i8(a, r.stream);
        };
        B.step(std::move(s));
    };
    auto move_last_step_after_producer = [&](int tensor_id) {
        int pos = 0;
        for (int i = (int)h->steps.size() - 2; i >= 0 && !pos; i--)
            for (int t : h->steps[i].out) if (t == tensor_id) { pos = i + 1; break; }
        Step st = std::move(h->steps.back());
        h->steps.pop_back();
        h->steps.insert(h->steps.begin() + pos, std::move(st));
    };
    auto ssh = [&](const std::string &lvname, int tin, int fh, int fw, int level, int lane) {
        const std::string p = "rf_" + lvname + "_det";
        int cat = B.tensor(p + "_concat_relu", fh, fw, 64);
        int ctx1 = B.tensor(p + "_context_conv1_relu", fh, fw, 16);
        int ctx31 = B.tensor(p + "_context_conv3_1_relu", fh, fw, 16);
        conv_step("ssh_" + lvname + "_conv1+ctx1_3x3_64to48", {&m.conv(p + "_conv1"), &m.conv(p + "_context_conv1")}, tin, fh, fw, cat, 64, 0, 32, 1,
                  ctx1, 16, 0, 1, lane, -1, 0, -1);
        conv_step("ssh_" + lvname + "_ctx2+ctx3_1_3x3_16to32", {&m.conv(p + "_context_conv2"), &m.conv(p + "_context_conv3_1")}, ctx1, fh, fw, cat,
                  64, 32, 16, 1, ctx31, 16, 0, 1, lane, -1, 0, -1);
        conv_step("ssh_" + lvname + "_ctx3_2_3x3_16to16", {&m.conv(p + "_context_conv3_2")}, ctx31, fh, fw, cat, 64, 48, 16, 1, -1, 0, 0, 0, lane, -1,
                  0, -1);
        h->feat_tensor[level] = cat;
    };
    const int h32 = H / 32, w32 = W / 32, h16 = H / 16, w16 = W / 16, h8 = H / 8, w8 = W / 8;
    int lat3 = B.tensor("rf_c3_lateral_relu", h32, w32, 64);
    int lat2 = B.tensor("rf_c2_lateral_relu", h16, w16, 64);
    int lat1 = B.tensor("rf_c1_red_conv_relu", h8, w8, 64);
    conv_step("c1_red_1x1_64to64", {&m.conv("rf_c1_red_conv")}, c1, h8, w8, lat1, 64, 0, 64, 1, -1, 0, 0, 0, 1, -1, 0, -1);
    move_last_step_after_producer(c1);
    conv_step("c2_lateral_1x1_128to64", {&m.conv("rf_c2_lateral")}, c2, h16, w16, lat2, 64, 0, 64, 1, -1, 0, 0, 0, 2, -1, 0, -1);
    move_last_step_after_producer(c2);
    conv_step("c3_lateral_1x1_256to64", {&m.conv("rf_c3_lateral")}, c3, h32, w32, lat3, 64, 0, 64, 1, -1, 0, 0, 0, 0, -1, 0, -1);
    ssh("c3", lat3, h32, w32, 0, 1);
    int aggr2 = B.tensor("rf_c2_aggr_relu", h16, w16, 64);
    conv_step("c2_upsample+add+aggr_3x3_64to64", {&m.conv("rf_c2_aggr")}, lat2, h16, w16, aggr2, 64, 0, 64, 1, -1, 0, 0, 0, 0, lat3, 0, lat2);
    ssh("c2", aggr2, h16, w16, 1, 2);
    int aggr1 = B.tensor("rf_c1_aggr_relu", h8, w8, 64);
    const long c1_tiles = ((long)h->cfg.max_batch * (h8 + 1) * (w8 + 2) + 127) / 128;
    if (c1_tiles <= h->num_sms) {
        conv_step("c1_upsample+add+aggr_3x3_64to64", {&m.conv("rf_c1_aggr")}, lat1, h8, w8, aggr1, 64, 0, 64, 1, -1, 0, 0, 0, 0, aggr2, 1, lat1);
    } else {
        int plus1 = B.tensor("_plus1", h8, w8, 64);
        const float s_out = tscale(plus1), s_up = tscale(aggr2), s_lat = tscale(lat1);
        std::vector<float> wq(16 * 64);
        for (int c = 0; c < 64; c++)
            for (int t = 0; t < 16; t++) wq[t * 64 + c] = (float)((double)m.up_w[1][c * 16 + t] * (double)s_up / (double)s_out);
        size_t owq = B.add_weights(wq);
        const float lat_mul = (float)((double)s_lat / (double)s_out);
        Step s;
        s.name = "i8_fpn_merge_c1_upsample+add";
        s.in = {lat1, aggr2}; s.out = {plus1};
        s.flops_per_img = 2.0 * h8 * w8 * 64 * 4;
        s.bytes_per_img = (double)h8 * w8 * 64 * 2 + (double)(h8 / 2) * (w8 / 2) * 64;
        s.launch = [=](const Run &r) {
            launch_k(k_fpn_merge_i8, dim3((unsigned)((w8 * 4 + 127) / 128), (unsigned)h8, (unsigned)r.n), dim3(128), 0, r.stream, (const int8_t *)Q_(r, lat1), (const int8_t *)Q_(r, aggr2), Q_(r, plus1),
                     Wd(owq), lat_mul, r.n, h8, w8, 64);
        };
        B.step(std::move(s));
        conv_step("c1_aggr_3x3_64to64", {&m.conv("rf_c1_aggr")}, plus1, h8, w8, aggr1, 64, 0, 64, 1, -1, 0, 0, 0, 0, -1, 0, -1);
    }
    ssh("c1", aggr1, h8, w8, 2, 0);
    size_t hw_off[3], hb_off[3];
    float hs[3];
    const int strides[3] = {32, 16, 8};
    for (int l = 0; l < 3; l++) {
        std::string st = "_stride" + std::to_string(strides[l]);
        const FoldedConv *cs[3] = {&m.conv("face_rpn_cls_score" + st), &m.conv("face_rpn_bbox_pred" + st), &m.conv("face_rpn_landmark_pred" + st)};
        std::vector<float> w(32 * 64), b(32);
        int r = 0;
        for (auto c : cs)
            for (int o = 0; o < c->cout; o++, r++) {
                b[r] = c->b[o];
                for (int ci = 0; ci < 64; ci++) w[r * 64 + ci] = c->w[(size_t)o * 64 + ci];
            }
        hw_off[l] = B.add_weights(w);
        hb_off[l] = B.add_weights(b);
        hs[l] = tscale(h->feat_tensor[l]);
    }
    {
        Step s;
        s.name = "i8_heads_1x1+softmax+decode_all_levels";
        s.in = {h->feat_tensor[0], h->feat_tensor[1], h->feat_tensor[2]};
        double px = (double)h32 * w32 + (double)h16 * w16 + (double)h8 * w8;
        s.flops_per_img = 2.0 * px * 64 * 4;
        s.bytes_per_img = px * 64;
        int f0 = h->feat_tensor[0], f1 = h->feat_tensor[1], f2 = h->feat_tensor[2];
        size_t w0 = hw_off[0], w1 = hw_off[1], w2 = hw_off[2], b0 = hb_off[0], b1 = hb_off[1], b2 = hb_off[2];
        float s0 = hs[0], s1 = hs[1], s2 = hs[2];
        s.launch = [=](const Run &r) {
            const int8_t *feat[3] = {Q_(r, f0), Q_(r, f1), Q_(r, f2)};
            HeadWeights hws[3] = {{Wd(w0), Wd(b0), s0}, {Wd(w1), Wd(b1), s1}, {Wd(w2), Wd(b2), s2}};
            launch_head_decode<int8_t>(feat, hws, h->lv, r.n, W, H, r.ctx.d_params, r.ctx.pb, r.blobs, r.stream, true);
        };
        s.name = "i8_heads_1x1+softmax+decode+nms_all_levels";
        h->head_step = (int)h->steps.size();
        B.step(std::move(s));
    }
}

}
```

retinaface_b200/csrc/stem_tc.cuh:

```cuda
#pragma once
#include "tc_conv.cuh"

namespace rf {

constexpr int STEM_B0_BYTES = 2 * 4 * 16 * 8 * 2, STEM_B1_BYTES = 2 * 16 * 8 * 2, STEM_F_FLOATS = 8 + 72 + 8 + 16 + 128;
constexpr int STEM_CONST_BYTES = STEM_B0_BYTES + STEM_B1_BYTES + STEM_F_FLOATS * 4;
static_assert(STEM_CONST_BYTES % 16 == 0, "bulk copy size");
struct StemTcArgs {
    const unsigned char *consts;
};

constexpr int STEM_LBO0 = 384 * 16 + 16;
constexpr int STEM_LBO1 = 256 * 16 + 16;

template <typename OutT>
__global__ void __launch_bounds__(256, 4) k_stem_tc(const PostParams *__restrict__ run, OutT *__restrict__ out, StemTcArgs w,
                                                    int n, int H, int W, float out_inv_scale) {
    constexpr bool I8 = sizeof(OutT) == 1;
    __shared__ __align__(16) uint8_t s_in[37][116];
    __shared__ __align__(128) unsigned char s_a0[4 * STEM_LBO0];
    __shared__ __align__(128) unsigned char s_const[STEM_CONST_BYTES];
    __shared__ __align__(8) uint64_t bar_w;

    unsigned char *s_a1 = s_a0;
    constexpr int STEM_C0_OFF = (2 * STEM_LBO1 + 127) / 128 * 128;
    static_assert(STEM_C0_OFF + 18 * 18 * 8 * 4 <= 4 * STEM_LBO0, "conv0 ring must fit behind the pointwise operand");
    float (*s_c0)[18 * 18][4] = reinterpret_cast<float (*)[18 * 18][4]>(s_a0 + STEM_C0_OFF);
    const int tid = threadIdx.x, warp = tid >> 5, lane = tid & 31;
    const int OH = H >> 1, OW = W >> 1;
    const int b = blockIdx.z;
    const int oy0 = blockIdx.y << 4, ox0 = blockIdx.x << 4;

    const __half *s_b0 = reinterpret_cast<const __half *>(s_const), *s_b1 = reinterpret_cast<const __half *>(s_const + STEM_B0_BYTES);
    const float *s_bias0 = reinterpret_cast<const float *>(s_const + STEM_B0_BYTES + STEM_B1_BYTES);
    const float *s_wd = s_bias0 + 8, *s_bias2 = s_bias0 + 8 + 72 + 8;
    if (tid == 0) {
        tc::mbar_init(&bar_w, 1);
        asm volatile("fence.mbarrier_init.release.cluster;" ::: "memory");
        tc::mbar_expect_tx(&bar_w, STEM_CONST_BYTES);
        tc::bulk_g2s(s_const, w.consts, STEM_CONST_BYTES, &bar_w);
    }
    pdl_trigger();
    pdl_wait();
    const uint8_t *__restrict__ img = run->input + (size_t)b * H * W * 3;
    const int iy0 = 2 * oy0 - 3, cb0 = (2 * ox0 - 3) * 3;
    const int al0 = cb0 & ~3, mis = cb0 - al0;
    const bool aligned = ((reinterpret_cast<uintptr_t>(img) & 3) == 0);
    const int rowbytes = W * 3;
    {
        uint32_t v[5];
        const int gb = al0 + 4 * lane;
        const bool fast = aligned && gb >= 0 && gb + 3 < rowbytes;
#pragma unroll
        for (int k = 0; k < 5; k++) {
            const int r = warp + 8 * k, iy = iy0 + r;
            v[k] = 0;
            if (r < 37 && lane < 29 && iy >= 0 && iy < H) {
                const uint8_t *rowp = img + (size_t)iy * rowbytes;
                if (fast) {
                    v[k] = __ldg(reinterpret_cast<const uint32_t *>(rowp + gb));
                } else {
#pragma unroll
                    for (int j = 0; j < 4; j++)
                        if (gb + j >= 0 && gb + j < rowbytes) v[k] |= (uint32_t)rowp[gb + j] << (8 * j);
                }
            }
        }
#pragma unroll
        for (int k = 0; k < 5; k++) {
            const int r = warp + 8 * k;
            if (r < 37 && lane < 29) *reinterpret_cast<uint32_t *>(&s_in[r][4 * lane]) = v[k];
        }
    }
    __syncthreads();
    for (int p = tid; p < 384; p += 256) {
        uint32_t h2[16];
#pragma unroll
        for (int i = 0; i < 16; i++) h2[i] = 0;
        if (p < 324) {
            const int py = p / 18, px = p - py * 18;
            const int off = mis + 6 * px, sh = (off & 3) * 8;
            uint32_t bytes[3][3];
#pragma unroll
            for (int ky = 0; ky < 3; ky++) {
                const uint32_t *row = reinterpret_cast<const uint32_t *>(&s_in[2 * py + ky][off & ~3]);
                const uint32_t w0 = row[0], w1 = row[1], w2 = row[2];
                bytes[ky][0] = __funnelshift_r(w0, w1, sh);
                bytes[ky][1] = __funnelshift_r(w1, w2, sh);
                bytes[ky][2] = __funnelshift_r(w2, 0u, sh);
            }
            const __half2 k1024 = __floats2half2_rn(1024.f, 1024.f);
#pragma unroll
            for (int i = 0; i < 14; i++) {
                const int k0 = 2 * i, k1 = 2 * i + 1 < 27 ? 2 * i + 1 : 2 * i;
                const int ra = k0 / 9, ja = k0 % 9, rb = k1 / 9, jb = k1 % 9;
                const uint32_t wa = bytes[ra][ja >> 2], wb = bytes[rb][jb >> 2];
                uint32_t biased;
                if (ra == rb && (ja >> 2) == (jb >> 2))
                    biased = __byte_perm(wa, 0x64646464u, (ja & 3) | 0x40 | ((jb & 3) << 8) | 0x4000);
                else
                    biased = __byte_perm(__byte_perm(wa, wb, (ja & 3) | ((4 + (jb & 3)) << 4)), 0x64646464u, 0x4140);
                const __half2 r = __hsub2(*reinterpret_cast<const __half2 *>(&biased), k1024);
                h2[i] = *reinterpret_cast<const uint32_t *>(&r);
            }
            h2[13] &= 0xffffu;
        }
#pragma unroll
        for (int g = 0; g < 4; g++)
            *reinterpret_cast<uint4 *>(s_a0 + g * STEM_LBO0 + p * 16) = make_uint4(h2[4 * g], h2[4 * g + 1], h2[4 * g + 2], h2[4 * g + 3]);
    }
    tc::fence_async_smem();
    __syncthreads();
    tc::mbar_wait(&bar_w, 0);
    const int wgi = warp >> 2, c2 = 2 * (lane & 3);
    const int rl = 16 * (warp & 3) + (lane >> 2);
    float d0[3][8];
    {
        const uint32_t a0 = tc::smem_u32(s_a0), b0 = tc::smem_u32(s_b0);
#pragma unroll
        for (int j = 0; j < 3; j++)
#pragma unroll
            for (int i = 0; i < 8; i++) d0[j][i] = 0.f;
        wg::fence();
#pragma unroll
        for (int j = 0; j < 3; j++)
#pragma unroll
            for (int part = 0; part < 2; part++)
#pragma unroll
                for (int ks = 0; ks < 2; ks++) {
                    const uint64_t ad = wg::desc(a0 + (uint32_t)(2 * ks) * STEM_LBO0 + (uint32_t)(64 * (wgi + 2 * j)) * 16, STEM_LBO0, 128);
                    const uint64_t bd = wg::desc(b0 + (uint32_t)(part * 4 + 2 * ks) * 256, 256, 128);
                    wg::mma_ss<16>(d0[j], ad, bd, part | ks);
                }
        wg::commit();
        wg::wait<0>();
#pragma unroll
        for (int j = 0; j < 3; j++) wg::fence_regs(d0[j]);
    }
    __syncthreads();
#pragma unroll
    for (int j = 0; j < 3; j++)
#pragma unroll
        for (int e = 0; e < 2; e++) {
            const int p = 64 * (wgi + 2 * j) + rl + 8 * e;
            if (p < 324) {
                const int py = p / 18, px = p - py * 18;
                const int cy = oy0 - 1 + py, cx = ox0 - 1 + px;
                const bool inside = cy >= 0 && cy < OH && cx >= 0 && cx < OW;
                const float v0 = inside ? fmaxf(d0[j][2 * e] + s_bias0[c2], 0.f) : 0.f;
                const float v1 = inside ? fmaxf(d0[j][2 * e + 1] + s_bias0[c2 + 1], 0.f) : 0.f;
                *reinterpret_cast<float2 *>(&s_c0[c2 >> 2][p][c2 & 3]) = make_float2(v0, v1);
            }
        }
    __syncthreads();
    {
        const int plane = tid >> 7, q = tid & 127;
        const int tx = q & 15, ty = (q >> 4) << 1;
        const float4 bv = *reinterpret_cast<const float4 *>(&s_wd[72 + plane * 4]);
        float d0[4] = {bv.x, bv.y, bv.z, bv.w}, d1[4] = {bv.x, bv.y, bv.z, bv.w};
#pragma unroll
        for (int ry = 0; ry < 4; ry++)
#pragma unroll
            for (int kx = 0; kx < 3; kx++) {
                const float4 a = *reinterpret_cast<const float4 *>(&s_c0[plane][(ty + ry) * 18 + tx + kx][0]);
                if (ry < 3) {
                    const float4 w = *reinterpret_cast<const float4 *>(&s_wd[(ry * 3 + kx) * 8 + plane * 4]);
                    d0[0] = fmaf(a.x, w.x, d0[0]); d0[1] = fmaf(a.y, w.y, d0[1]); d0[2] = fmaf(a.z, w.z, d0[2]); d0[3] = fmaf(a.w, w.w, d0[3]);
                }
                if (ry > 0) {
                    const float4 w = *reinterpret_cast<const float4 *>(&s_wd[((ry - 1) * 3 + kx) * 8 + plane * 4]);
                    d1[0] = fmaf(a.x, w.x, d1[0]); d1[1] = fmaf(a.y, w.y, d1[1]); d1[2] = fmaf(a.z, w.z, d1[2]); d1[3] = fmaf(a.w, w.w, d1[3]);
                }
            }
        const int row = ty * 16 + tx;
        if constexpr (I8) {
            float (*s_dwo)[256][4] = reinterpret_cast<float (*)[256][4]>(s_a1);
            *reinterpret_cast<float4 *>(&s_dwo[plane][row][0]) = make_float4(fmaxf(d0[0], 0.f), fmaxf(d0[1], 0.f), fmaxf(d0[2], 0.f), fmaxf(d0[3], 0.f));
            *reinterpret_cast<float4 *>(&s_dwo[plane][row + 16][0]) = make_float4(fmaxf(d1[0], 0.f), fmaxf(d1[1], 0.f), fmaxf(d1[2], 0.f), fmaxf(d1[3], 0.f));
        } else {
            const __half2 h00 = __floats2half2_rn(fmaxf(d0[0], 0.f), fmaxf(d0[1], 0.f)), h01 = __floats2half2_rn(fmaxf(d0[2], 0.f), fmaxf(d0[3], 0.f));
            const __half2 h10 = __floats2half2_rn(fmaxf(d1[0], 0.f), fmaxf(d1[1], 0.f)), h11 = __floats2half2_rn(fmaxf(d1[2], 0.f), fmaxf(d1[3], 0.f));
            *reinterpret_cast<uint2 *>(s_a1 + row * 16 + plane * 8) = make_uint2(*reinterpret_cast<const uint32_t *>(&h00), *reinterpret_cast<const uint32_t *>(&h01));
            *reinterpret_cast<uint2 *>(s_a1 + (row + 16) * 16 + plane * 8) = make_uint2(*reinterpret_cast<const uint32_t *>(&h10), *reinterpret_cast<const uint32_t *>(&h11));
            *reinterpret_cast<uint4 *>(s_a1 + STEM_LBO1 + tid * 16) = make_uint4(0, 0, 0, 0);
        }
    }
    if constexpr (I8) {
        __syncthreads();
        const float (*s_dwo)[256][4] = reinterpret_cast<const float (*)[256][4]>(s_a1);
        const float *s_wp = s_bias2 + 16;
        const int oy = oy0 + (tid >> 4), ox = ox0 + (tid & 15);
        if (oy < OH && ox < OW) {
            const float4 da = *reinterpret_cast<const float4 *>(&s_dwo[0][tid][0]), db = *reinterpret_cast<const float4 *>(&s_dwo[1][tid][0]);
            const float d[8] = {da.x, da.y, da.z, da.w, db.x, db.y, db.z, db.w};
            float o[16];
#pragma unroll
            for (int j = 0; j < 16; j++) o[j] = s_bias2[j];
#pragma unroll
            for (int c = 0; c < 8; c++)
#pragma unroll
                for (int j4 = 0; j4 < 4; j4++) {
                    const float4 wv = *reinterpret_cast<const float4 *>(&s_wp[c * 16 + j4 * 4]);
                    o[j4 * 4 + 0] = fmaf(d[c], wv.x, o[j4 * 4 + 0]); o[j4 * 4 + 1] = fmaf(d[c], wv.y, o[j4 * 4 + 1]);
                    o[j4 * 4 + 2] = fmaf(d[c], wv.z, o[j4 * 4 + 2]); o[j4 * 4 + 3] = fmaf(d[c], wv.w, o[j4 * 4 + 3]);
                }
            uint32_t pk[4];
#pragma unroll
            for (int j4 = 0; j4 < 4; j4++) {
                uint32_t word = 0;
#pragma unroll
                for (int k = 0; k < 4; k++) {
                    int q = __float2int_rn(__fmul_rn(fmaxf(o[j4 * 4 + k], 0.f), out_inv_scale));
                    q = max(-127, min(127, q));
                    word |= (uint32_t)(q & 0xff) << (8 * k);
                }
                pk[j4] = word;
            }
            *reinterpret_cast<uint4 *>(out + (((size_t)b * OH + oy) * OW + ox) * 16) = make_uint4(pk[0], pk[1], pk[2], pk[3]);
        }
    } else {
    tc::fence_async_smem();
    __syncthreads();
    float d1[2][8];
    {
        const uint32_t a1 = tc::smem_u32(s_a1), b1 = tc::smem_u32(s_b1);
#pragma unroll
        for (int j = 0; j < 2; j++)
#pragma unroll
            for (int i = 0; i < 8; i++) d1[j][i] = 0.f;
        wg::fence();
#pragma unroll
        for (int j = 0; j < 2; j++)
            wg::mma_ss<16>(d1[j], wg::desc(a1 + (uint32_t)(64 * (wgi + 2 * j)) * 16, STEM_LBO1, 128), wg::desc(b1, 256, 128), 0);
        wg::commit();
        wg::wait<0>();
#pragma unroll
        for (int j = 0; j < 2; j++) wg::fence_regs(d1[j]);
    }
#pragma unroll
    for (int j = 0; j < 2; j++)
#pragma unroll
        for (int e = 0; e < 2; e++) {
            const int row = 64 * (wgi + 2 * j) + rl + 8 * e;
            const int oy = oy0 + (row >> 4), ox = ox0 + (row & 15);
            if (oy < OH && ox < OW) {
                __half *dst = reinterpret_cast<__half *>(out) + (((size_t)b * OH + oy) * OW + ox) * 16;
#pragma unroll
                for (int i = 0; i < 2; i++) {
                    const int c = 8 * i + c2;
                    *reinterpret_cast<__half2 *>(dst + c) = __floats2half2_rn(fmaxf(d1[j][4 * i + 2 * e] + s_bias2[c], 0.f),
                                                                              fmaxf(d1[j][4 * i + 2 * e + 1] + s_bias2[c + 1], 0.f));
                }
            }
        }
    }
}

}
```

retinaface_b200/csrc/tc_conv.cuh:

```cuda
#pragma once
#include "common.cuh"
#include "wgmma.cuh"

namespace rf {

constexpr int TC_LBO_A = 128 * 16 + 16;

struct TcOut {
    __half *p0; int ld0; int n0; int relu0;
    __half *p1; int ld1; int relu1;
};

namespace tc {

__device__ __forceinline__ uint32_t smem_u32(const void *p) { return (uint32_t)__cvta_generic_to_shared(p); }

__device__ __forceinline__ void mbar_init(uint64_t *bar, unsigned count) {
    asm volatile("mbarrier.init.shared::cta.b64 [%0], %1;" ::"r"(smem_u32(bar)), "r"(count));
}
__device__ __forceinline__ void mbar_expect_tx(uint64_t *bar, unsigned bytes) {
    asm volatile("mbarrier.arrive.expect_tx.shared::cta.b64 _, [%0], %1;" ::"r"(smem_u32(bar)), "r"(bytes) : "memory");
}
__device__ __forceinline__ void mbar_wait(uint64_t *bar, unsigned parity) {
    unsigned done = 0;
    unsigned spins = 0;
    while (!done) {
        asm volatile(
            "{\n\t.reg .pred p;\n\t"
            "mbarrier.try_wait.parity.shared::cta.b64 p, [%1], %2;\n\t"
            "selp.u32 %0, 1, 0, p;\n\t}"
            : "=r"(done)
            : "r"(smem_u32(bar)), "r"(parity)
            : "memory");
        if (!done && ++spins > (1u << 24)) __trap();
    }
}
__device__ __forceinline__ void bulk_g2s(void *dst, const void *src, unsigned bytes, uint64_t *bar) {
    asm volatile("cp.async.bulk.shared::cluster.global.mbarrier::complete_tx::bytes [%0], [%1], %2, [%3];" ::"r"(smem_u32(dst)),
                 "l"(src), "r"(bytes), "r"(smem_u32(bar))
                 : "memory");
}
__device__ __forceinline__ void fence_async_smem() { asm volatile("fence.proxy.async.shared::cta;" ::: "memory"); }

}

constexpr int tc_n_bucket(int n) { return n <= 32 ? 32 : (n <= 64 ? 64 : (n <= 128 ? 128 : 256)); }

constexpr int TC_THREADS = 256;
constexpr int TC_MAX_R = 2048;

struct TcConvArgs {
    const __half *in;
    int Cin, nimg, H, W;
    int taps;
    int N;
    int Wp, Hp;
    int R;
    uint32_t mul_Wp, mul_Hp, mul_H;
    const __half *wimg;
    const float *bias;
    TcOut out;
    const __half *up;
    const float *up_w;
    int Cmax;
};

__device__ __forceinline__ void cp_async16_zfill(void *smem_dst, const void *gsrc, bool valid) {
    const unsigned sz = valid ? 16u : 0u;
    asm volatile("cp.async.cg.shared.global [%0], [%1], 16, %2;" ::"r"(tc::smem_u32(smem_dst)), "l"(gsrc), "r"(sz) : "memory");
}
__device__ __forceinline__ void cp_async16_zfill_s(uint32_t smem_dst, const void *gsrc, bool valid) {
    const unsigned sz = valid ? 16u : 0u;
    asm volatile("cp.async.cg.shared.global [%0], [%1], 16, %2;" ::"r"(smem_dst), "l"(gsrc), "r"(sz) : "memory");
}
__device__ __forceinline__ void cp_async_wait_all() {
    asm volatile("cp.async.commit_group;\n\tcp.async.wait_group 0;" ::: "memory");
}

__device__ __forceinline__ int tc_frag_row() { return 64 * (threadIdx.x >> 7) + 16 * ((threadIdx.x >> 5) & 3) + ((threadIdx.x & 31) >> 2); }

template <int NC>
__device__ __forceinline__ void tc_epilogue(const float (&d)[NC / 2], int n0, const float *s_bias ,
                                            const TcOut &o, const long (&out_row)[2], int n_off) {
    const int c2 = 2 * (threadIdx.x & 3);
#pragma unroll
    for (int e = 0; e < 2; e++) {
        if (out_row[e] < 0) continue;
#pragma unroll
        for (int i = 0; i < NC / 8; i++) {
            const int n = n0 + 8 * i + c2;
            const int gn = n_off + n;
            const bool first = gn < o.n0;
            const int relu = first ? o.relu0 : o.relu1;
            __half *dst = first ? o.p0 + (size_t)out_row[e] * o.ld0 + gn : o.p1 + (size_t)out_row[e] * o.ld1 + (gn - o.n0);
            float f0 = d[4 * i + 2 * e] + s_bias[n], f1 = d[4 * i + 2 * e + 1] + s_bias[n + 1];
            if (relu) { f0 = fmaxf(f0, 0.f); f1 = fmaxf(f1, 0.f); }
            *reinterpret_cast<__half2 *>(dst) = __floats2half2_rn(f0, f1);
        }
    }
}

inline size_t tc_conv_smem_bytes(const TcConvArgs &a) {
    return (size_t)(a.Cin / 8) * a.R * 16 + (size_t)a.taps * a.Cin * a.N * 2 + (a.up ? (size_t)(a.Cin / 8) * a.Cmax * 16 : 0) +
           (size_t)a.R * 4 * (a.up ? 2 : 1) + 128;
}

template <int NT, bool UPADD>
__global__ void __launch_bounds__(TC_THREADS) k_tc_conv_staged(const TcConvArgs a) {
    extern __shared__ __align__(128) unsigned char smem[];
    __shared__ __align__(8) uint64_t bar_b;
    __shared__ float s_bias[256];
    __shared__ __align__(16) __half s_uw[UPADD ? 64 * 16 : 8];
    __shared__ int s_crow[2];

    const int tid = threadIdx.x, warp = tid >> 5;
    const int pad = a.taps == 9 ? 1 : 0;
    const int G = a.Cin >> 3;
    const uint32_t lbo_s = (uint32_t)a.R * 16;
    unsigned char *sS = smem;
    unsigned char *sB = smem + (size_t)G * lbo_s;
    int *s_off = reinterpret_cast<int *>(sB + (size_t)a.taps * a.Cin * a.N * 2 + (UPADD ? (size_t)G * a.Cmax * 16 : 0));
    int *s_yx = s_off + a.R;
    const int m0 = blockIdx.x * 128;
    const int lo = m0 - (a.Wp + 1) * pad;

    if (tid == 0) {
        s_crow[0] = 0x7fffffff; s_crow[1] = -1;
        tc::mbar_init(&bar_b, 1);
        asm volatile("fence.mbarrier_init.release.cluster;" ::: "memory");
        const unsigned bytes = (unsigned)((size_t)a.taps * a.Cin * a.N * 2);
        tc::mbar_expect_tx(&bar_b, bytes);
        tc::bulk_g2s(sB, a.wimg, bytes, &bar_b);
    }
    pdl_trigger();
    if (tid < a.N) s_bias[tid] = a.bias[tid];
    if (UPADD) for (int i = tid; i < a.Cin * 16; i += TC_THREADS) s_uw[(i & 15) * 64 + (i >> 4)] = __float2half_rn(a.up_w[i]);
    {
        const int lane = tid & 31;
        const int prow0 = fast_floor_div(lo, a.Wp, a.mul_Wp);
        const int prow1 = fast_div(lo + a.R - 1, a.mul_Wp);
        for (int prow = prow0 + warp; prow <= prow1; prow += TC_THREADS / 32) {
            const int b = prow >= 0 ? fast_div(prow, a.mul_Hp) : -1;
            const int yy = prow >= 0 ? (int)(prow - b * a.Hp) : 0;
            const bool rowok = prow >= 0 && b < a.nimg && yy < a.H;
            for (int xx = lane; xx < a.Wp; xx += 32) {
                const int pl = prow * a.Wp + xx - lo;
                if (pl < 0 || pl >= a.R) continue;
                int off = -1;
                if (rowok && xx >= pad && xx < a.W + pad) {
                    off = ((b * a.H + yy) * a.W + (xx - pad)) * a.Cin;
                    if (UPADD) {
                        s_yx[pl] = ((b * a.H + yy) << 12) | (xx - pad);
                        const int UH = a.H >> 1, ih = (yy + 1) >> 1;
                        atomicMin(&s_crow[0], b * UH + max(ih - 1, 0));
                        atomicMax(&s_crow[1], b * UH + min(ih, UH - 1));
                    }
                }
                s_off[pl] = off;
            }
        }
    }
    __syncthreads();
    pdl_wait();
    const int lg = 31 - __clz(G);
    const int UH = a.H >> 1, UW = a.W >> 1;
    unsigned char *sC = sB + (size_t)a.taps * a.Cin * a.N * 2;
    const int crow_lo = UPADD ? s_crow[0] : 0, crow_hi = UPADD ? s_crow[1] : -1;
    if (UPADD && crow_hi >= crow_lo) {
        const int ncp = (crow_hi - crow_lo + 1) * UW;
        if (ncp > a.Cmax) __trap();
        const __half *csrc = a.up + (size_t)crow_lo * UW * a.Cin;
        for (int it = tid; it < ncp * G; it += TC_THREADS) cp_async16_zfill(sC + (size_t)it * 16, csrc + (size_t)it * 8, true);
    }
    {
        constexpr int UNR = 4;
        const int g = tid & (G - 1), p0 = tid >> lg, pstep = TC_THREADS >> lg;
        const __half *src_g = a.in + g * 8;
        unsigned char *dst_g = sS + (uint32_t)g * lbo_s;
        for (int pb = p0; pb < a.R; pb += pstep * UNR) {
            uint4 v[UNR];
#pragma unroll
            for (int u = 0; u < UNR; u++) {
                const int p = pb + u * pstep;
                v[u] = make_uint4(0, 0, 0, 0);
                if (p < a.R) {
                    const int off = s_off[p];
                    if (off >= 0) v[u] = __ldcg(reinterpret_cast<const uint4 *>(src_g + off));
                }
            }
#pragma unroll
            for (int u = 0; u < UNR; u++) {
                const int p = pb + u * pstep;
                if (p < a.R) *reinterpret_cast<uint4 *>(dst_g + (uint32_t)p * 16u) = v[u];
            }
        }
    }
    if (UPADD) {
        cp_async_wait_all();
        __syncthreads();
        for (int it = tid; it < a.R * G; it += TC_THREADS) {
            const int g = it & (G - 1), pl = it >> lg;
            const int off = s_off[pl];
            if (off < 0) continue;
            const int c0 = g * 8;
            const int yx = s_yx[pl];
            const int x = yx & 0xfff, gy = yx >> 12;
            const int b = fast_div(gy, a.mul_H), y = gy - b * a.H;
            unsigned char *slot = sS + (size_t)g * lbo_s + (size_t)pl * 16;
            uint4 accv = *reinterpret_cast<const uint4 *>(slot);
            __half2 *acc = reinterpret_cast<__half2 *>(&accv);
            const int i_hi = (y + 1) >> 1, j_hi = (x + 1) >> 1;
#pragma unroll
            for (int di = 0; di < 2; di++) {
                const int i = i_hi - di, ky = y - 2 * i + 1;
                if (i < 0 || i >= UH || ky < 0 || ky > 3) continue;
#pragma unroll
                for (int dj = 0; dj < 2; dj++) {
                    const int j = j_hi - dj, kx = x - 2 * j + 1;
                    if (j < 0 || j >= UW || kx < 0 || kx > 3) continue;
                    const uint4 uv = *reinterpret_cast<const uint4 *>(sC + ((size_t)((b * UH + i - crow_lo) * UW + j) * G + g) * 16);
                    const uint4 wv = *reinterpret_cast<const uint4 *>(&s_uw[(ky * 4 + kx) * 64 + c0]);
                    const __half2 *u2 = reinterpret_cast<const __half2 *>(&uv), *w2 = reinterpret_cast<const __half2 *>(&wv);
#pragma unroll
                    for (int c = 0; c < 4; c++) acc[c] = __hfma2(u2[c], w2[c], acc[c]);
                }
            }
            *reinterpret_cast<uint4 *>(slot) = accv;
        }
    } else {
        cp_async_wait_all();
    }
    tc::fence_async_smem();
    __syncthreads();
    tc::mbar_wait(&bar_b, 0);
    const int row_base = (int)(m0 - lo);
    long orow[2];
#pragma unroll
    for (int e = 0; e < 2; e++) {
        const int off = s_off[row_base + tc_frag_row() + 8 * e];
        orow[e] = off >= 0 ? (off >> (31 - __clz(a.Cin))) : -1;
    }
    const uint32_t s_addr = tc::smem_u32(sS) + (uint32_t)(row_base + 64 * (warp >> 2)) * 16u, b_addr = tc::smem_u32(sB);
    const uint32_t lbo_b = (uint32_t)a.N * 16;
    wg::for_chunks<(NT < 64 ? NT : 64)>(a.N, [&](auto nc, int n0) {
        constexpr int NC = decltype(nc)::value;
        float d[NC / 2];
        wg::fence();
        int acc = 0;
        for (int t = 0; t < a.taps; t++) {
            const int shift = pad ? (t / 3 - 1) * a.Wp + (t % 3 - 1) : 0;
            for (int cs = 0; cs < (a.Cin >> 4); cs++) {
                const uint64_t ad = wg::desc(s_addr + (uint32_t)(2 * cs) * lbo_s + (uint32_t)(shift * 16), lbo_s, 128);
                const uint64_t bd = wg::desc(b_addr + (uint32_t)(t * G + 2 * cs) * lbo_b + (uint32_t)n0 * 16u, lbo_b, 128);
                wg::mma_ss<NC>(d, ad, bd, acc);
                acc = 1;
            }
        }
        wg::commit();
        wg::wait<0>();
        wg::fence_regs(d);
        tc_epilogue<NC>(d, n0, s_bias, a.out, orow, 0);
    });
}

struct TcDwArgs {
    const __half *in;
    int C, nimg, IH, IW, OH, OW, S;
    int N;
    int Ntotal;
    int Kpad;
    int rows;
    int Wp, Hp;
    int Rmax;
    uint32_t mul_Wp, mul_Hp, mul_OW, mul_OH;
    const __half *wimg;
    const float *bias;
    const float *dw_w, *dw_b;
    __half *out;
};

__host__ __device__ inline uint32_t tc_dw_lbo_a(int rows) { return (uint32_t)rows * 16 + 16; }
inline size_t tc_dw_smem_bytes(const TcDwArgs &a) {
    return (size_t)((a.C + 7) / 8) * a.Rmax * 16 + (size_t)(a.Kpad / 8) * tc_dw_lbo_a(a.rows) + (size_t)a.Kpad * a.N * 2 +
           (size_t)10 * a.C * 4 + (size_t)a.Rmax * 4 + 128;
}

template <int NT>
__global__ void __launch_bounds__(TC_THREADS, 3) k_tc_dwpw_staged(const TcDwArgs a) {
    extern __shared__ __align__(128) unsigned char smem[];
    __shared__ __align__(8) uint64_t bar_b;
    __shared__ int s_cpos[128];
    __shared__ float s_bias[256];

    const int tid = threadIdx.x, warp = tid >> 5;
    const int G = a.C >> 3;
    const int GA = a.Kpad >> 3;
    const int lgGA = 31 - __clz(GA);
    const int g_own = tid & (GA - 1);
    const int pix = a.C * 2;
    unsigned char *sS = smem;
    unsigned char *sA = smem + (size_t)a.Rmax * pix;
    const uint32_t lbo_a = tc_dw_lbo_a(a.rows);
    unsigned char *sB = sA + (size_t)(a.Kpad / 8) * lbo_a;
    float *s_dww = reinterpret_cast<float *>(sB + (size_t)a.Kpad * a.N * 2);
    float *s_dwb = s_dww + 9 * a.C;
    int *s_off = reinterpret_cast<int *>(s_dwb + a.C);
    const int M = a.nimg * a.OH * a.OW;
    const int m0 = blockIdx.x * a.rows;
    const int mlast = min(m0 + a.rows, M) - 1;
    auto centre = [&](int m) -> int {
        const int q = fast_div(m, a.mul_OW), ox = m - q * a.OW, b = fast_div(q, a.mul_OH), oy = q - b * a.OH;
        return (b * a.Hp + oy * a.S) * a.Wp + ox * a.S + 1;
    };
    const int lo = centre(m0) - a.Wp - 1;
    const int R = (int)(centre(mlast) + a.Wp + 1 - lo) + 1;
    if (R > a.Rmax) __trap();

    if (tid == 0) {
        tc::mbar_init(&bar_b, 1);
        asm volatile("fence.mbarrier_init.release.cluster;" ::: "memory");
        const unsigned bytes = (unsigned)((size_t)a.Kpad * a.N * 2);
        tc::mbar_expect_tx(&bar_b, bytes);
        tc::bulk_g2s(sB, a.wimg + (size_t)blockIdx.y * a.Kpad * a.N, bytes, &bar_b);
    }
    pdl_trigger();
    if (tid < a.N) s_bias[tid] = a.bias[blockIdx.y * a.N + tid];
    for (int i = tid; i < 9 * a.C; i += TC_THREADS) s_dww[i] = dw_weight_f16(a.dw_w[i]);
    for (int i = tid; i < a.C; i += TC_THREADS) s_dwb[i] = a.dw_b[i];
    {
        const int lane = tid & 31;
        const int prow0 = fast_floor_div(lo, a.Wp, a.mul_Wp);
        const int prow1 = fast_div(lo + R - 1, a.mul_Wp);
        for (int prow = prow0 + warp; prow <= prow1; prow += TC_THREADS / 32) {
            const int b = prow >= 0 ? fast_div(prow, a.mul_Hp) : -1;
            const int yy = prow >= 0 ? (int)(prow - b * a.Hp) : 0;
            const bool rowok = prow >= 0 && b < a.nimg && yy < a.IH;
            for (int xx = lane; xx < a.Wp; xx += 32) {
                const int pl = prow * a.Wp + xx - lo;
                if (pl < 0 || pl >= R) continue;
                s_off[pl] = (rowok && xx >= 1 && xx <= a.IW) ? ((b * a.IH + yy) * a.IW + (xx - 1)) * a.C : -1;
            }
        }
    }
    if (tid < 128) {
        const int m = m0 + tid;
        s_cpos[tid] = (tid < a.rows && m < M) ? (int)(centre(m) - lo) : -1;
    }
    __syncthreads();
    pdl_wait();
    const int lg = 31 - __clz(G);
    {
        const uint32_t sS_s = tc::smem_u32(sS);
        const __half *src_g = a.in + (tid & (G - 1)) * 8;
        for (int it = tid; it < R * G; it += TC_THREADS) {
            const int off = s_off[it >> lg];
            cp_async16_zfill_s(sS_s + (uint32_t)it * 16u, off >= 0 ? src_g + off : a.in, off >= 0);
        }
    }
    cp_async_wait_all();
    __syncthreads();
    if (g_own < G) {
        auto stencil = [&](auto s_) {
            constexpr int S = decltype(s_)::value;
            const float *w = s_dww + g_own * 8;
            const int win = g_own * 16 - (a.Wp + 1) * pix;
            for (int r0 = 4 * (tid >> lgGA); r0 < a.rows; r0 += 4 * (TC_THREADS >> lgGA)) {
                const int cp0 = s_cpos[r0];
                if (cp0 < 0) continue;
                unsigned char *dst = sA + (size_t)g_own * lbo_a + (size_t)r0 * 16;
                if (s_cpos[r0 + 3] == cp0 + 3 * S) {
                    float acc[1][4][8];
                    dw_bias8(acc[0][0], s_dwb + g_own * 8);
#pragma unroll
                    for (int i = 0; i < 8; i++) { acc[0][1][i] = acc[0][0][i]; acc[0][2][i] = acc[0][0][i]; acc[0][3][i] = acc[0][0][i]; }
                    dw_stencil_block<S, 1, 4>(acc, sS + win + cp0 * pix, a.Wp * pix, pix, w, a.C);
#pragma unroll
                    for (int q = 0; q < 4; q++) *reinterpret_cast<uint4 *>(dst + q * 16) = dw_relu_h8(acc[0][q]);
// ... 50 lines not shown
```

retinaface_b200/csrc/tc_dwpw2d.cuh:

```cuda
#pragma once
#include "tc_conv.cuh"

namespace rf {

struct TcDw2dArgs {
    const __half *in;
    int C, nimg, IH, IW, OH, OW, S;
    int N;
    int TH, TW;
    int tiles_x, tiles_y;
    int PH, PW;
    uint32_t lbo_a;
    uint32_t mul_TW, mul_tiles_x, mul_tiles;
    const __half *wimg;
    const float *bias;
    const float *dw_w, *dw_b;
    __half *out;
};

inline void tc_dw2d_finish(TcDw2dArgs &a) {
    const int G = a.C >> 3;
    a.PH = (a.TH - 1) * a.S + 3;
    a.PW = (a.TW - 1) * a.S + 3;
    a.tiles_x = (a.OW + a.TW - 1) / a.TW;
    a.tiles_y = (a.OH + a.TH - 1) / a.TH;
    a.lbo_a = (uint32_t)(128 + 8 / G) * 16;
    a.mul_TW = fast_div_mul((uint32_t)a.TW);
    a.mul_tiles_x = fast_div_mul((uint32_t)a.tiles_x);
    a.mul_tiles = fast_div_mul((uint32_t)(a.tiles_x * a.tiles_y));
}
inline size_t tc_dw2d_smem_bytes(const TcDw2dArgs &a) {
    return (size_t)a.PH * a.PW * a.C * 2 + (size_t)(a.C / 8) * a.lbo_a + (size_t)a.C * a.N * 2 + 128;
}

#ifndef RF_DW2D_OCC
#define RF_DW2D_OCC 3
#endif
template <int NT>
__global__ void __launch_bounds__(TC_THREADS, RF_DW2D_OCC) k_tc_dwpw_2d(const TcDw2dArgs a) {
    extern __shared__ __align__(128) unsigned char smem[];
    __shared__ __align__(8) uint64_t bar_b;
    __shared__ float s_bias[256];
    __shared__ __align__(16) float s_dww[9 * 64];
    __shared__ __align__(16) float s_dwb[64];

    const int tid = threadIdx.x, warp = tid >> 5, lane = tid & 31;
    const int G = a.C >> 3, lg = 31 - __clz(G);
    const int PH = a.PH, PW = a.PW;
    const uint32_t lbo_a = a.lbo_a;
    const int pix = a.C * 2;
    unsigned char *sS = smem;
    unsigned char *sA = smem + (size_t)PH * PW * pix;
    unsigned char *sB = sA + (size_t)G * lbo_a;
    const int tiles = a.tiles_x * a.tiles_y;
    const int b = fast_div((int)blockIdx.x, a.mul_tiles), trem = blockIdx.x - b * tiles;
    const int ty0 = fast_div(trem, a.mul_tiles_x);
    const int oy0 = ty0 * a.TH, ox0 = (trem - ty0 * a.tiles_x) * a.TW;
    const int iy0 = oy0 * a.S - 1, ix0 = ox0 * a.S - 1;

    if (tid == 0) {
        tc::mbar_init(&bar_b, 1);
        asm volatile("fence.mbarrier_init.release.cluster;" ::: "memory");
        const unsigned bytes = (unsigned)((size_t)a.C * a.N * 2);
        tc::mbar_expect_tx(&bar_b, bytes);
        tc::bulk_g2s(sB, a.wimg, bytes, &bar_b);
    }
    pdl_trigger();
    if (tid < a.N) s_bias[tid] = a.bias[tid];
    for (int i = tid; i < 9 * a.C; i += TC_THREADS) s_dww[i] = dw_weight_f16(a.dw_w[i]);
    if (tid < a.C) s_dwb[tid] = a.dw_b[tid];
    pdl_wait();
    {
        const int per_row = PW << lg;
        const int px_lo = max(0, -ix0), px_hi = min(PW, a.IW - ix0);
        const unsigned px_n = (unsigned)max(px_hi - px_lo, 0);
        const uint32_t sS_s = tc::smem_u32(sS);
        for (int py = warp; py < PH; py += TC_THREADS / 32) {
            const int iy = iy0 + py;
            const bool rowok = iy >= 0 && iy < a.IH;
            const __half *src_row = a.in + (ptrdiff_t)(((b * a.IH + (rowok ? iy : 0)) * a.IW + ix0) * a.C);
            const uint32_t dst_row = sS_s + (uint32_t)(py * PW * pix);
            const __half *zsrc = a.in;
            for (int i = lane; i < per_row; i += 32) {
                const bool ok = rowok && (unsigned)((i >> lg) - px_lo) < px_n;
                cp_async16_zfill_s(dst_row + (uint32_t)i * 16u, ok ? src_row + i * 8 : zsrc, ok);
            }
        }
    }
    cp_async_wait_all();
    __syncthreads();
    const int rows = a.TH * a.TW;
    auto stencil = [&](auto s_) {
        constexpr int S = decltype(s_)::value;
        const int items = (a.TH >> 1) * (a.TW >> 1) << lg;
        for (int it = tid; it < items; it += TC_THREADS) {
            const int g = it & (G - 1), rest = it >> lg;
            const int typ = fast_div(2 * rest, a.mul_TW), ty = 2 * typ, tx = 2 * rest - typ * a.TW;
            float acc[2][2][8];
            dw_bias8(acc[0][0], &s_dwb[g * 8]);
#pragma unroll
            for (int i = 0; i < 8; i++) { acc[0][1][i] = acc[0][0][i]; acc[1][0][i] = acc[0][0][i]; acc[1][1][i] = acc[0][0][i]; }
            dw_stencil_block<S, 2, 2>(acc, sS + (ty * S * PW + tx * S) * pix + g * 16, PW * pix, pix, &s_dww[g * 8], a.C);
            const int r = ty * a.TW + tx;
            unsigned char *dst = sA + (size_t)g * lbo_a + (size_t)r * 16;
            *reinterpret_cast<uint4 *>(dst) = dw_relu_h8(acc[0][0]);
            *reinterpret_cast<uint4 *>(dst + 16) = dw_relu_h8(acc[0][1]);
            *reinterpret_cast<uint4 *>(dst + a.TW * 16) = dw_relu_h8(acc[1][0]);
            *reinterpret_cast<uint4 *>(dst + a.TW * 16 + 16) = dw_relu_h8(acc[1][1]);
        }
    };
    if (a.S == 1) stencil(std::integral_constant<int, 1>{});
    else stencil(std::integral_constant<int, 2>{});
    tc::fence_async_smem();
    __syncthreads();
    if (64 * (warp >> 2) >= rows) return;
    tc::mbar_wait(&bar_b, 0);
    long orow[2];
#pragma unroll
    for (int e = 0; e < 2; e++) {
        const int r = tc_frag_row() + 8 * e;
        const int ty = fast_div(r, a.mul_TW), tx = r - ty * a.TW;
        const int oy = oy0 + ty, ox = ox0 + tx;
        orow[e] = (r < rows && oy < a.OH && ox < a.OW) ? (long)((b * a.OH + oy) * a.OW + ox) : -1;
    }
    const uint32_t a_addr = tc::smem_u32(sA) + (uint32_t)(64 * (warp >> 2)) * 16u, b_addr = tc::smem_u32(sB);
    const uint32_t lbo_b = (uint32_t)a.N * 16;
    const TcOut o{a.out, a.N, a.N, 1, nullptr, 0, 0};
    wg::for_chunks<(NT < 32 ? NT : 32)>(a.N, [&](auto nc, int n0) {
        constexpr int NC = decltype(nc)::value;
        float d[NC / 2];
        wg::fence();
        wg::mma_ss<NC>(d, wg::desc(a_addr, lbo_a, 128), wg::desc(b_addr + (uint32_t)n0 * 16u, lbo_b, 128), 0);
        for (int ks = 1; ks < (a.C >> 4); ks++) {
            const uint64_t ad = wg::desc(a_addr + (uint32_t)(2 * ks) * lbo_a, lbo_a, 128);
            const uint64_t bd = wg::desc(b_addr + (uint32_t)(2 * ks) * lbo_b + (uint32_t)n0 * 16u, lbo_b, 128);
            wg::mma_ss<NC>(d, ad, bd, 1);
        }
        wg::commit();
        wg::wait<0>();
        wg::fence_regs(d);
        tc_epilogue<NC>(d, n0, s_bias, o, orow, 0);
    });
}

}
```

Baseline: 319,500.

## Make stem and 2D dw+pw kernels persistent with double-buffered cp.async tile staging

Converts the tensor-core stem kernel and the 2D depthwise+pointwise kernel into persistent kernels. Each CTA loops over a contiguous run of tiles sized from occupancy-derived resident CTA counts, and prefetches the next tile's input into a second shared-memory buffer with cp.async while computing the current one. This amortises per-CTA setup (weight loads, barrier init, B-matrix bulk copy) and hides global load latency. The cost is doubled input staging shared memory, which may lower occupancy. The dw stencil is also reshaped from 2x2 to 1x2 output blocks per item.

Measured after the change: 342,800 (median of 6 runs). 1.07x the previous value.

```diff
diff --git a/retinaface_b200/csrc/engine.cu b/retinaface_b200/csrc/engine.cu
--- a/retinaface_b200/csrc/engine.cu
+++ b/retinaface_b200/csrc/engine.cu
@@ -84,6 +84,7 @@
 void make_plan(rf_handle h, bool init) {
     const rf_config &cfg = h->cfg;
     h->use_tc = cfg.precision == RF_PREC_INT8 || (cfg.precision == RF_PREC_FP16 && !(cfg.flags & RF_FLAG_NO_TENSORCORE));
+    h->on_device = init;
     if (init && h->use_tc) CK(tc_init());
     if (cfg.precision == RF_PREC_INT8) { if (init) CK(tc_init_i8()); build_plan_i8(h); }
     else if (cfg.precision == RF_PREC_FP32) build_plan<float>(h);
diff --git a/retinaface_b200/csrc/engine_internal.cuh b/retinaface_b200/csrc/engine_internal.cuh
--- a/retinaface_b200/csrc/engine_internal.cuh
+++ b/retinaface_b200/csrc/engine_internal.cuh
@@ -112,6 +112,7 @@
     std::map<std::string, float> int8_scales;
     int device = 0;
     int num_sms = RF_NUM_SMS;
+    bool on_device = false;
     int elem = 4;
     cudaEvent_t ev0 = nullptr, ev1 = nullptr;
 
@@ -225,6 +226,12 @@
 std::vector<__half> make_stem_blob(const std::vector<float> &w0, const std::vector<float> &b0, const std::vector<float> &wd,
                                    const std::vector<float> &bd, const std::vector<float> &wp, const std::vector<float> &bp);
 int plan_stem_tc(Builder &B);
+int resident_ctas(rf_handle h, const void *kern, int threads, size_t smem);
+struct PersistentGrid { int run, grid; };
+inline PersistentGrid persistent_grid(int tiles, int resident) {
+    const int run = std::max(1, (tiles + resident - 1) / std::max(resident, 1));
+    return {run, (tiles + run - 1) / run};
+}
 int plan_pair_legacy(Builder &B, int i, int tin, int ih, int iw);
 void plan_conv_legacy(Builder &B, const std::string &sname, std::vector<const FoldedConv *> cs, int tin, int ih, int iw, int t0, int ld0,
                       int off0, int n0, int relu0, int t1, int ld1, int off1, int relu1, int lane = 0, int tup = -1, int up_which = 0);
diff --git a/retinaface_b200/csrc/plan_fp.cu b/retinaface_b200/csrc/plan_fp.cu
--- a/retinaface_b200/csrc/plan_fp.cu
+++ b/retinaface_b200/csrc/plan_fp.cu
@@ -92,15 +92,26 @@
         default: CK_L(k_tc_dwpw_staged<256>, grid, dim3(TC_THREADS), smem, s, a); break;
     }
 }
-void launch_tc_dwpw_2d(const TcDw2dArgs &a, cudaStream_t s) {
-    const dim3 grid((unsigned)(a.tiles_x * a.tiles_y * a.nimg));
-    const size_t smem = tc_dw2d_smem_bytes(a);
-    switch (tc_n_bucket(a.N)) {
-        case 32: CK_L(k_tc_dwpw_2d<32>, grid, dim3(TC_THREADS), smem, s, a); break;
-        case 64: CK_L(k_tc_dwpw_2d<64>, grid, dim3(TC_THREADS), smem, s, a); break;
-        case 128: CK_L(k_tc_dwpw_2d<128>, grid, dim3(TC_THREADS), smem, s, a); break;
-        default: CK_L(k_tc_dwpw_2d<256>, grid, dim3(TC_THREADS), smem, s, a); break;
-    }
+static void (*dw2d_kernel(int N))(TcDw2dArgs) {
+    switch (tc_n_bucket(N)) {
+        case 32: return k_tc_dwpw_2d<32>;
+        case 64: return k_tc_dwpw_2d<64>;
+        case 128: return k_tc_dwpw_2d<128>;
+        default: return k_tc_dwpw_2d<256>;
+    }
+}
+void launch_tc_dwpw_2d(TcDw2dArgs a, int resident, cudaStream_t s) {
+    const PersistentGrid pg = persistent_grid(a.tiles_x * a.tiles_y * a.nimg, resident);
+    a.run = pg.run;
+    CK_L(dw2d_kernel(a.N), dim3((unsigned)pg.grid), dim3(TC_THREADS), tc_dw2d_smem_bytes(a), s, a);
+}
+
+int resident_ctas(rf_handle h, const void *kern, int threads, size_t smem) {
+    if (!h->on_device) return h->num_sms;
+    int per_sm = 0;
+    CK(cudaOccupancyMaxActiveBlocksPerMultiprocessor(&per_sm, kern, threads, smem));
+    if (per_sm < 1) throw PlanFail{RF_ERR_UNSUPPORTED, fmt("a kernel with %zu bytes of dynamic shared memory does not fit an SM", smem)};
+    return per_sm * h->num_sms;
 }
 
 cudaError_t tc_init() {
@@ -192,17 +203,23 @@
     s.flops_per_img = 2.0 * oh * ow_ * C * 9 + 2.0 * oh * ow_ * C * N;
     s.bytes_per_img = ((double)ih * iw * C + (double)oh * ow_ * N) * es;
     const bool tiles2d = oh * ow_ > 56 * 56 && C >= 16 && C <= 64 && geo.nsplit == 1 && !(h->cfg.flags & RF_FLAG_DW_1D);
-    if (tiles2d) s.name = fmt("tc2d_dw%d+pw%d_s%d_%dto%d", i, i + 1, S, C, N);
+    TcDw2dArgs g2{};
+    int resident = 0;
+    if (tiles2d) {
+        s.name = fmt("tc2d_dw%d+pw%d_s%d_%dto%d", i, i + 1, S, C, N);
+        g2.C = C; g2.IH = ih; g2.IW = iw; g2.OH = oh; g2.OW = ow_; g2.S = S; g2.N = N;
+        g2.TH = 8;
+        const int t16 = (ow_ + 15) / 16, t14 = (ow_ + 13) / 14;
+        g2.TW = t14 < t16 ? 14 : 16;
+        tc_dw2d_finish(g2);
+        resident = resident_ctas(h, (const void *)dw2d_kernel(N), TC_THREADS, tc_dw2d_smem_bytes(g2));
+    }
     s.launch = [=](const Run &r) {
         if (tiles2d) {
-            TcDw2dArgs a{};
-            a.in = T_(r, tin); a.C = C; a.nimg = r.n; a.IH = ih; a.IW = iw; a.OH = oh; a.OW = ow_; a.S = S; a.N = N;
-            a.TH = 8;
-            const int t16 = (ow_ + 15) / 16, t14 = (ow_ + 13) / 14;
-            a.TW = t14 < t16 ? 14 : 16;
-            tc_dw2d_finish(a);
+            TcDw2dArgs a = g2;
+            a.in = T_(r, tin); a.nimg = r.n;
             a.wimg = h->d_weights_h + oimg; a.bias = Wd(obp); a.dw_w = Wd(owd); a.dw_b = Wd(obd); a.out = T_(r, tpw);
-            launch_tc_dwpw_2d(a, r.stream);
+            launch_tc_dwpw_2d(a, resident, r.stream);
             return;
         }
         TcDwArgs a{};
@@ -365,14 +382,17 @@
     s.out = {out};
     s.flops_per_img = 2.0 * cur_h * cur_w * (8 * 27 + 8 * 9 + 8 * 16);
     s.bytes_per_img = (double)H * W * 3 + (double)cur_h * cur_w * 16 * es;
+    const int tiles = ((H / 2 + 15) / 16) * ((W / 2 + 15) / 16);
+    const int resident = simt_stem ? 0 : resident_ctas(h, (const void *)k_stem_tc<__half>, 256, 0);
     s.launch = [=](const Run &r) {
-        const int tiles = ((H / 2 + 15) / 16) * ((W / 2 + 15) / 16);
         if (simt_stem) {
             StemWeights sw{Wd(ow0), Wd(ob0), Wd(owd), Wd(obd), Wd(owp), Wd(obp)};
             CK(launch_k(k_stem<__half>, dim3((unsigned)(tiles * r.n)), dim3(256), 0, r.stream, (const PostParams *)r.ctx.d_params, (__half *)T_(r, out), sw, r.n, H, W, 1.0f));
         } else {
             StemTcArgs a{reinterpret_cast<const unsigned char *>(h->d_weights_h + oblob)};
-            CK(launch_k(k_stem_tc<__half>, dim3((unsigned)((W / 2 + 15) / 16), (unsigned)((H / 2 + 15) / 16), (unsigned)r.n), dim3(256), 0, r.stream, (const PostParams *)r.ctx.d_params, (__half *)T_(r, out), a, r.n, H, W, 1.0f));
+            const PersistentGrid pg = persistent_grid(tiles * r.n, resident);
+            stem_tc_finish(a, H, W, pg.run);
+            CK(launch_k(k_stem_tc<__half>, dim3((unsigned)pg.grid), dim3(256), 0, r.stream, (const PostParams *)r.ctx.d_params, (__half *)T_(r, out), a, r.n, H, W, 1.0f));
         }
     };
     B.step(std::move(s));
diff --git a/retinaface_b200/csrc/plan_i8.cu b/retinaface_b200/csrc/plan_i8.cu
--- a/retinaface_b200/csrc/plan_i8.cu
+++ b/retinaface_b200/csrc/plan_i8.cu
@@ -152,14 +152,17 @@
         const bool simt_stem = (h->cfg.flags & (RF_FLAG_SIMT_STEM | RF_FLAG_NO_TENSORCORE)) != 0;
         size_t oblob = B.add_weights_h(make_stem_blob(w0, c0.b, wd, dw.b, wp, pw.b));
         if (!simt_stem) s.name = "tc_stem_conv0+dw1+pw2_u8_to_16ch_i8";
+        const int tiles = ((H / 2 + 15) / 16) * ((W / 2 + 15) / 16);
+        const int resident = simt_stem ? 0 : resident_ctas(h, (const void *)k_stem_tc<int8_t>, 256, 0);
         s.launch = [=](const Run &r) {
             if (simt_stem) {
                 StemWeights sw{Wd(ow0), Wd(ob0), Wd(owd), Wd(obd), Wd(owp), Wd(obp)};
-                const int tiles = ((H / 2 + 15) / 16) * ((W / 2 + 15) / 16);
                 launch_k(k_stem<int8_t>, dim3((unsigned)(tiles * r.n)), dim3(256), 0, r.stream, (const PostParams *)r.ctx.d_params, Q_(r, out), sw, r.n, H, W, inv);
             } else {
                 StemTcArgs a{reinterpret_cast<const unsigned char *>(h->d_weights_h + oblob)};
-                launch_k(k_stem_tc<int8_t>, dim3((unsigned)((W / 2 + 15) / 16), (unsigned)((H / 2 + 15) / 16), (unsigned)r.n), dim3(256), 0, r.stream,
+                const PersistentGrid pg = persistent_grid(tiles * r.n, resident);
+                stem_tc_finish(a, H, W, pg.run);
+                launch_k(k_stem_tc<int8_t>, dim3((unsigned)pg.grid), dim3(256), 0, r.stream,
                          (const PostParams *)r.ctx.d_params, Q_(r, out), a, r.n, H, W, inv);
             }
         };
diff --git a/retinaface_b200/csrc/stem_tc.cuh b/retinaface_b200/csrc/stem_tc.cuh
--- a/retinaface_b200/csrc/stem_tc.cuh
+++ b/retinaface_b200/csrc/stem_tc.cuh
@@ -8,7 +8,15 @@
 static_assert(STEM_CONST_BYTES % 16 == 0, "bulk copy size");
 struct StemTcArgs {
     const unsigned char *consts;
+    int tiles_per_cta;
+    uint32_t mul_tiles, mul_tiles_x;
 };
+inline void stem_tc_finish(StemTcArgs &a, int H, int W, int tiles_per_cta) {
+    const int tiles_x = (W / 2 + 15) / 16, tiles = tiles_x * ((H / 2 + 15) / 16);
+    a.tiles_per_cta = tiles_per_cta;
+    a.mul_tiles = fast_div_mul((uint32_t)tiles);
+    a.mul_tiles_x = fast_div_mul((uint32_t)tiles_x);
+}
 
 constexpr int STEM_LBO0 = 384 * 16 + 16;
 constexpr int STEM_LBO1 = 256 * 16 + 16;
@@ -17,7 +25,7 @@
 __global__ void __launch_bounds__(256, 4) k_stem_tc(const PostParams *__restrict__ run, OutT *__restrict__ out, StemTcArgs w,
                                                     int n, int H, int W, float out_inv_scale) {
     constexpr bool I8 = sizeof(OutT) == 1;
-    __shared__ __align__(16) uint8_t s_in[37][116];
+    __shared__ __align__(16) uint8_t s_in[2][37][116];
     __shared__ __align__(128) unsigned char s_a0[4 * STEM_LBO0];
     __shared__ __align__(128) unsigned char s_const[STEM_CONST_BYTES];
     __shared__ __align__(8) uint64_t bar_w;
@@ -28,8 +36,13 @@
     float (*s_c0)[18 * 18][4] = reinterpret_cast<float (*)[18 * 18][4]>(s_a0 + STEM_C0_OFF);
     const int tid = threadIdx.x, warp = tid >> 5, lane = tid & 31;
     const int OH = H >> 1, OW = W >> 1;
-    const int b = blockIdx.z;
-    const int oy0 = blockIdx.y << 4, ox0 = blockIdx.x << 4;
+    const int tiles_x = (OW + 15) >> 4, tiles = tiles_x * ((OH + 15) >> 4);
+    const int t_begin = (int)blockIdx.x * w.tiles_per_cta, t_end = min(t_begin + w.tiles_per_cta, tiles * n);
+    auto decode = [&](int t, int &b, int &oy0, int &ox0) {
+        b = fast_div(t, w.mul_tiles);
+        const int trem = t - b * tiles, ty = fast_div(trem, w.mul_tiles_x);
+        oy0 = ty << 4; ox0 = (trem - ty * tiles_x) << 4;
+    };
 
     const __half *s_b0 = reinterpret_cast<const __half *>(s_const), *s_b1 = reinterpret_cast<const __half *>(s_const + STEM_B0_BYTES);
     const float *s_bias0 = reinterpret_cast<const float *>(s_const + STEM_B0_BYTES + STEM_B1_BYTES);
@@ -42,214 +55,223 @@
     }
     pdl_trigger();
     pdl_wait();
-    const uint8_t *__restrict__ img = run->input + (size_t)b * H * W * 3;
-    const int iy0 = 2 * oy0 - 3, cb0 = (2 * ox0 - 3) * 3;
-    const int al0 = cb0 & ~3, mis = cb0 - al0;
-    const bool aligned = ((reinterpret_cast<uintptr_t>(img) & 3) == 0);
-    const int rowbytes = W * 3;
-    {
-        uint32_t v[5];
-        const int gb = al0 + 4 * lane;
-        const bool fast = aligned && gb >= 0 && gb + 3 < rowbytes;
-#pragma unroll
-        for (int k = 0; k < 5; k++) {
-            const int r = warp + 8 * k, iy = iy0 + r;
-            v[k] = 0;
-            if (r < 37 && lane < 29 && iy >= 0 && iy < H) {
-                const uint8_t *rowp = img + (size_t)iy * rowbytes;
-                if (fast) {
-                    v[k] = __ldg(reinterpret_cast<const uint32_t *>(rowp + gb));
+    auto stage = [&](int t, int buf) {
+        int b, oy0, ox0;
+        decode(t, b, oy0, ox0);
+        const uint8_t *__restrict__ img = run->input + (size_t)b * H * W * 3;
+        const int iy0 = 2 * oy0 - 3, cb0 = (2 * ox0 - 3) * 3;
+        const int gb = (cb0 & ~3) + 4 * lane;
+        const int rowbytes = W * 3;
+        const bool fast = ((reinterpret_cast<uintptr_t>(img) & 3) == 0) && gb >= 0 && gb + 3 < rowbytes;
+        if (lane < 29) {
+#pragma unroll
+            for (int k = 0; k < 5; k++) {
+                const int r = warp + 8 * k, iy = iy0 + r;
+                if (r >= 37) break;
+                uint8_t *dst = &s_in[buf][r][4 * lane];
+                const bool rowok = iy >= 0 && iy < H;
+                const uint8_t *rowp = img + (size_t)(rowok ? iy : 0) * rowbytes;
+                if (fast && rowok) {
+                    cp_async4(dst, rowp + gb);
                 } else {
-#pragma unroll
-                    for (int j = 0; j < 4; j++)
-                        if (gb + j >= 0 && gb + j < rowbytes) v[k] |= (uint32_t)rowp[gb + j] << (8 * j);
-                }
-            }
-        }
-#pragma unroll
-        for (int k = 0; k < 5; k++) {
-            const int r = warp + 8 * k;
-            if (r < 37 && lane < 29) *reinterpret_cast<uint32_t *>(&s_in[r][4 * lane]) = v[k];
-        }
-    }
-    __syncthreads();
-    for (int p = tid; p < 384; p += 256) {
-        uint32_t h2[16];
-#pragma unroll
-        for (int i = 0; i < 16; i++) h2[i] = 0;
-        if (p < 324) {
-            const int py = p / 18, px = p - py * 18;
-            const int off = mis + 6 * px, sh = (off & 3) * 8;
-            uint32_t bytes[3][3];
-#pragma unroll
-            for (int ky = 0; ky < 3; ky++) {
-                const uint32_t *row = reinterpret_cast<const uint32_t *>(&s_in[2 * py + ky][off & ~3]);
-                const uint32_t w0 = row[0], w1 = row[1], w2 = row[2];
-                bytes[ky][0] = __funnelshift_r(w0, w1, sh);
-                bytes[ky][1] = __funnelshift_r(w1, w2, sh);
-                bytes[ky][2] = __funnelshift_r(w2, 0u, sh);
-            }
-            const __half2 k1024 = __floats2half2_rn(1024.f, 1024.f);
-#pragma unroll
-            for (int i = 0; i < 14; i++) {
-                const int k0 = 2 * i, k1 = 2 * i + 1 < 27 ? 2 * i + 1 : 2 * i;
-                const int ra = k0 / 9, ja = k0 % 9, rb = k1 / 9, jb = k1 % 9;
-                const uint32_t wa = bytes[ra][ja >> 2], wb = bytes[rb][jb >> 2];
-                uint32_t biased;
-                if (ra == rb && (ja >> 2) == (jb >> 2))
-                    biased = __byte_perm(wa, 0x64646464u, (ja & 3) | 0x40 | ((jb & 3) << 8) | 0x4000);
-                else
-                    biased = __byte_perm(__byte_perm(wa, wb, (ja & 3) | ((4 + (jb & 3)) << 4)), 0x64646464u, 0x4140);
-                const __half2 r = __hsub2(*reinterpret_cast<const __half2 *>(&biased), k1024);
-                h2[i] = *reinterpret_cast<const uint32_t *>(&r);
-            }
-            h2[13] &= 0xffffu;
-        }
-#pragma unroll
-        for (int g = 0; g < 4; g++)
-            *reinterpret_cast<uint4 *>(s_a0 + g * STEM_LBO0 + p * 16) = make_uint4(h2[4 * g], h2[4 * g + 1], h2[4 * g + 2], h2[4 * g + 3]);
-    }
-    tc::fence_async_smem();
-    __syncthreads();
-    tc::mbar_wait(&bar_w, 0);
-    const int wgi = warp >> 2, c2 = 2 * (lane & 3);
-    const int rl = 16 * (warp & 3) + (lane >> 2);
-    float d0[3][8];
-    {
-        const uint32_t a0 = tc::smem_u32(s_a0), b0 = tc::smem_u32(s_b0);
-#pragma unroll
-        for (int j = 0; j < 3; j++)
-#pragma unroll
-            for (int i = 0; i < 8; i++) d0[j][i] = 0.f;
-        wg::fence();
-#pragma unroll
-        for (int j = 0; j < 3; j++)
-#pragma unroll
-            for (int part = 0; part < 2; part++)
-#pragma unroll
-                for (int ks = 0; ks < 2; ks++) {
-                    const uint64_t ad = wg::desc(a0 + (uint32_t)(2 * ks) * STEM_LBO0 + (uint32_t)(64 * (wgi + 2 * j)) * 16, STEM_LBO0, 128);
-                    const uint64_t bd = wg::desc(b0 + (uint32_t)(part * 4 + 2 * ks) * 256, 256, 128);
-                    wg::mma_ss<16>(d0[j], ad, bd, part | ks);
-                }
-        wg::commit();
-        wg::wait<0>();
-#pragma unroll
-        for (int j = 0; j < 3; j++) wg::fence_regs(d0[j]);
-    }
-    __syncthreads();
-#pragma unroll
-    for (int j = 0; j < 3; j++)
-#pragma unroll
-        for (int e = 0; e < 2; e++) {
-            const int p = 64 * (wgi + 2 * j) + rl + 8 * e;
+                    uint32_t v = 0;
+                    if (rowok)
+#pragma unroll
+                        for (int j = 0; j < 4; j++)
+                            if (gb + j >= 0 && gb + j < rowbytes) v |= (uint32_t)rowp[gb + j] << (8 * j);
+                    *reinterpret_cast<uint32_t *>(dst) = v;
+                }
+            }
+        }
+        cp_async_commit();
+    };
+    stage(t_begin, 0);
+    int buf = 0;
+    for (int t = t_begin; t < t_end; t++, buf ^= 1) {
+        cp_async_wait_all();
+        __syncthreads();
+        if (t + 1 < t_end) stage(t + 1, buf ^ 1);
+        int b, oy0, ox0;
+        decode(t, b, oy0, ox0);
+        const int mis = ((2 * ox0 - 3) * 3) & 3;
+        for (int p = tid; p < 384; p += 256) {
+            uint32_t h2[16];
+#pragma unroll
+            for (int i = 0; i < 16; i++) h2[i] = 0;
             if (p < 324) {
                 const int py = p / 18, px = p - py * 18;
-                const int cy = oy0 - 1 + py, cx = ox0 - 1 + px;
-                const bool inside = cy >= 0 && cy < OH && cx >= 0 && cx < OW;
-                const float v0 = inside ? fmaxf(d0[j][2 * e] + s_bias0[c2], 0.f) : 0.f;
-                const float v1 = inside ? fmaxf(d0[j][2 * e + 1] + s_bias0[c2 + 1], 0.f) : 0.f;
-                *reinterpret_cast<float2 *>(&s_c0[c2 >> 2][p][c2 & 3]) = make_float2(v0, v1);
-            }
-        }
-    __syncthreads();
-    {
-        const int plane = tid >> 7, q = tid & 127;
-        const int tx = q & 15, ty = (q >> 4) << 1;
-        const float4 bv = *reinterpret_cast<const float4 *>(&s_wd[72 + plane * 4]);
-        float d0[4] = {bv.x, bv.y, bv.z, bv.w}, d1[4] = {bv.x, bv.y, bv.z, bv.w};
-#pragma unroll
-        for (int ry = 0; ry < 4; ry++)
-#pragma unroll
-            for (int kx = 0; kx < 3; kx++) {
-                const float4 a = *reinterpret_cast<const float4 *>(&s_c0[plane][(ty + ry) * 18 + tx + kx][0]);
-                if (ry < 3) {
-                    const float4 w = *reinterpret_cast<const float4 *>(&s_wd[(ry * 3 + kx) * 8 + plane * 4]);
-                    d0[0] = fmaf(a.x, w.x, d0[0]); d0[1] = fmaf(a.y, w.y, d0[1]); d0[2] = fmaf(a.z, w.z, d0[2]); d0[3] = fmaf(a.w, w.w, d0[3]);
-                }
-                if (ry > 0) {
-                    const float4 w = *reinterpret_cast<const float4 *>(&s_wd[((ry - 1) * 3 + kx) * 8 + plane * 4]);
-                    d1[0] = fmaf(a.x, w.x, d1[0]); d1[1] = fmaf(a.y, w.y, d1[1]); d1[2] = fmaf(a.z, w.z, d1[2]); d1[3] = fmaf(a.w, w.w, d1[3]);
-                }
-            }
-        const int row = ty * 16 + tx;
+                const int off = mis + 6 * px, sh = (off & 3) * 8;
+                uint32_t bytes[3][3];
+#pragma unroll
+                for (int ky = 0; ky < 3; ky++) {
+                    const uint32_t *row = reinterpret_cast<const uint32_t *>(&s_in[buf][2 * py + ky][off & ~3]);
+                    const uint32_t w0 = row[0], w1 = row[1], w2 = row[2];
+                    bytes[ky][0] = __funnelshift_r(w0, w1, sh);
+                    bytes[ky][1] = __funnelshift_r(w1, w2, sh);
+                    bytes[ky][2] = __funnelshift_r(w2, 0u, sh);
+                }
+                const __half2 k1024 = __floats2half2_rn(1024.f, 1024.f);
+#pragma unroll
+                for (int i = 0; i < 14; i++) {
+                    const int k0 = 2 * i, k1 = 2 * i + 1 < 27 ? 2 * i + 1 : 2 * i;
+                    const int ra = k0 / 9, ja = k0 % 9, rb = k1 / 9, jb = k1 % 9;
+                    const uint32_t wa = bytes[ra][ja >> 2], wb = bytes[rb][jb >> 2];
+                    uint32_t biased;
+                    if (ra == rb && (ja >> 2) == (jb >> 2))
+                        biased = __byte_perm(wa, 0x64646464u, (ja & 3) | 0x40 | ((jb & 3) << 8) | 0x4000);
+                    else
+                        biased = __byte_perm(__byte_perm(wa, wb, (ja & 3) | ((4 + (jb & 3)) << 4)), 0x64646464u, 0x4140);
+                    const __half2 r = __hsub2(*reinterpret_cast<const __half2 *>(&biased), k1024);
+                    h2[i] = *reinterpret_cast<const uint32_t *>(&r);
+                }
+                h2[13] &= 0xffffu;
+            }
+#pragma unroll
+            for (int g = 0; g < 4; g++)
+                *reinterpret_cast<uint4 *>(s_a0 + g * STEM_LBO0 + p * 16) = make_uint4(h2[4 * g], h2[4 * g + 1], h2[4 * g + 2], h2[4 * g + 3]);
+        }
+        tc::fence_async_smem();
+        __syncthreads();
+        tc::mbar_wait(&bar_w, 0);
+        const int wgi = warp >> 2, c2 = 2 * (lane & 3);
+        const int rl = 16 * (warp & 3) + (lane >> 2);
+        float d0[3][8];
+        {
+            const uint32_t a0 = tc::smem_u32(s_a0), b0 = tc::smem_u32(s_b0);
+#pragma unroll
+            for (int j = 0; j < 3; j++)
+#pragma unroll
+                for (int i = 0; i < 8; i++) d0[j][i] = 0.f;
+            wg::fence();
+#pragma unroll
+            for (int j = 0; j < 3; j++)
+#pragma unroll
+                for (int part = 0; part < 2; part++)
+#pragma unroll
+                    for (int ks = 0; ks < 2; ks++) {
+                        const uint64_t ad = wg::desc(a0 + (uint32_t)(2 * ks) * STEM_LBO0 + (uint32_t)(64 * (wgi + 2 * j)) * 16, STEM_LBO0, 128);
+                        const uint64_t bd = wg::desc(b0 + (uint32_t)(part * 4 + 2 * ks) * 256, 256, 128);
+                        wg::mma_ss<16>(d0[j], ad, bd, part | ks);
+                    }
+            wg::commit();
+            wg::wait<0>();
+#pragma unroll
+            for (int j = 0; j < 3; j++) wg::fence_regs(d0[j]);
+        }
+        __syncthreads();
+#pragma unroll
+        for (int j = 0; j < 3; j++)
+#pragma unroll
+            for (int e = 0; e < 2; e++) {
+                const int p = 64 * (wgi + 2 * j) + rl + 8 * e;
+                if (p < 324) {
+                    const int py = p / 18, px = p - py * 18;
+                    const int cy = oy0 - 1 + py, cx = ox0 - 1 + px;
+                    const bool inside = cy >= 0 && cy < OH && cx >= 0 && cx < OW;
+                    const float v0 = inside ? fmaxf(d0[j][2 * e] + s_bias0[c2], 0.f) : 0.f;
+                    const float v1 = inside ? fmaxf(d0[j][2 * e + 1] + s_bias0[c2 + 1], 0.f) : 0.f;
+                    *reinterpret_cast<float2 *>(&s_c0[c2 >> 2][p][c2 & 3]) = make_float2(v0, v1);
+                }
+            }
+        __syncthreads();
+        {
+            const int plane = tid >> 7, q = tid & 127;
+            const int tx = q & 15, ty = (q >> 4) << 1;
+            const float4 bv = *reinterpret_cast<const float4 *>(&s_wd[72 + plane * 4]);
+            float d0[4] = {bv.x, bv.y, bv.z, bv.w}, d1[4] = {bv.x, bv.y, bv.z, bv.w};
+#pragma unroll
+            for (int ry = 0; ry < 4; ry++)
+#pragma unroll
+                for (int kx = 0; kx < 3; kx++) {
+                    const float4 a = *reinterpret_cast<const float4 *>(&s_c0[plane][(ty + ry) * 18 + tx + kx][0]);
+                    if (ry < 3) {
+                        const float4 w = *reinterpret_cast<const float4 *>(&s_wd[(ry * 3 + kx) * 8 + plane * 4]);
+                        d0[0] = fmaf(a.x, w.x, d0[0]); d0[1] = fmaf(a.y, w.y, d0[1]); d0[2] = fmaf(a.z, w.z, d0[2]); d0[3] = fmaf(a.w, w.w, d0[3]);
+                    }
+                    if (ry > 0) {
+                        const float4 w = *reinterpret_cast<const float4 *>(&s_wd[((ry - 1) * 3 + kx) * 8 + plane * 4]);
+                        d1[0] = fmaf(a.x, w.x, d1[0]); d1[1] = fmaf(a.y, w.y, d1[1]); d1[2] = fmaf(a.z, w.z, d1[2]); d1[3] = fmaf(a.w, w.w, d1[3]);
+                    }
+                }
+            const int row = ty * 16 + tx;
+            if constexpr (I8) {
+                float (*s_dwo)[256][4] = reinterpret_cast<float (*)[256][4]>(s_a1);
+                *reinterpret_cast<float4 *>(&s_dwo[plane][row][0]) = make_float4(fmaxf(d0[0], 0.f), fmaxf(d0[1], 0.f), fmaxf(d0[2], 0.f), fmaxf(d0[3], 0.f));
+                *reinterpret_cast<float4 *>(&s_dwo[plane][row + 16][0]) = make_float4(fmaxf(d1[0], 0.f), fmaxf(d1[1], 0.f), fmaxf(d1[2], 0.f), fmaxf(d1[3], 0.f));
+            } else {
+                const __half2 h00 = __floats2half2_rn(fmaxf(d0[0], 0.f), fmaxf(d0[1], 0.f)), h01 = __floats2half2_rn(fmaxf(d0[2], 0.f), fmaxf(d0[3], 0.f));
+                const __half2 h10 = __floats2half2_rn(fmaxf(d1[0], 0.f), fmaxf(d1[1], 0.f)), h11 = __floats2half2_rn(fmaxf(d1[2], 0.f), fmaxf(d1[3], 0.f));
+                *reinterpret_cast<uint2 *>(s_a1 + row * 16 + plane * 8) = make_uint2(*reinterpret_cast<const uint32_t *>(&h00), *reinterpret_cast<const uint32_t *>(&h01));
+                *reinterpret_cast<uint2 *>(s_a1 + (row + 16) * 16 + plane * 8) = make_uint2(*reinterpret_cast<const uint32_t *>(&h10), *reinterpret_cast<const uint32_t *>(&h11));
+                *reinterpret_cast<uint4 *>(s_a1 + STEM_LBO1 + tid * 16) = make_uint4(0, 0, 0, 0);
+            }
+        }
         if constexpr (I8) {
-            float (*s_dwo)[256][4] = reinterpret_cast<float (*)[256][4]>(s_a1);
-            *reinterpret_cast<float4 *>(&s_dwo[plane][row][0]) = make_float4(fmaxf(d0[0], 0.f), fmaxf(d0[1], 0.f), fmaxf(d0[2], 0.f), fmaxf(d0[3], 0.f));
-            *reinterpret_cast<float4 *>(&s_dwo[plane][row + 16][0]) = make_float4(fmaxf(d1[0], 0.f), fmaxf(d1[1], 0.f), fmaxf(d1[2], 0.f), fmaxf(d1[3], 0.f));
+            __syncthreads();
+            const float (*s_dwo)[256][4] = reinterpret_cast<const float (*)[256][4]>(s_a1);
+            const float *s_wp = s_bias2 + 16;
+            const int oy = oy0 + (tid >> 4), ox = ox0 + (tid & 15);
+            if (oy < OH && ox < OW) {
+                const float4 da = *reinterpret_cast<const float4 *>(&s_dwo[0][tid][0]), db = *reinterpret_cast<const float4 *>(&s_dwo[1][tid][0]);
+                const float d[8] = {da.x, da.y, da.z, da.w, db.x, db.y, db.z, db.w};
+                float o[16];
+#pragma unroll
+                for (int j = 0; j < 16; j++) o[j] = s_bias2[j];
+#pragma unroll
+                for (int c = 0; c < 8; c++)
+#pragma unroll
+                    for (int j4 = 0; j4 < 4; j4++) {
+                        const float4 wv = *reinterpret_cast<const float4 *>(&s_wp[c * 16 + j4 * 4]);
+                        o[j4 * 4 + 0] = fmaf(d[c], wv.x, o[j4 * 4 + 0]); o[j4 * 4 + 1] = fmaf(d[c], wv.y, o[j4 * 4 + 1]);
+                        o[j4 * 4 + 2] = fmaf(d[c], wv.z, o[j4 * 4 + 2]); o[j4 * 4 + 3] = fmaf(d[c], wv.w, o[j4 * 4 + 3]);
+                    }
+                uint32_t pk[4];
+#pragma unroll
+                for (int j4 = 0; j4 < 4; j4++) {
+                    uint32_t word = 0;
+#pragma unroll
+                    for (int k = 0; k < 4; k++) {
+                        int q = __float2int_rn(__fmul_rn(fmaxf(o[j4 * 4 + k], 0.f), out_inv_scale));
+                        q = max(-127, min(127, q));
+                        word |= (uint32_t)(q & 0xff) << (8 * k);
+                    }
+                    pk[j4] = word;
+                }
+                *reinterpret_cast<uint4 *>(out + (((size_t)b * OH + oy) * OW + ox) * 16) = make_uint4(pk[0], pk[1], pk[2], pk[3]);
+            }
         } else {
-            const __half2 h00 = __floats2half2_rn(fmaxf(d0[0], 0.f), fmaxf(d0[1], 0.f)), h01 = __floats2half2_rn(fmaxf(d0[2], 0.f), fmaxf(d0[3], 0.f));
-            const __half2 h10 = __floats2half2_rn(fmaxf(d1[0], 0.f), fmaxf(d1[1], 0.f)), h11 = __floats2half2_rn(fmaxf(d1[2], 0.f), fmaxf(d1[3], 0.f));
-            *reinterpret_cast<uint2 *>(s_a1 + row * 16 + plane * 8) = make_uint2(*reinterpret_cast<const uint32_t *>(&h00), *reinterpret_cast<const uint32_t *>(&h01));
-            *reinterpret_cast<uint2 *>(s_a1 + (row + 16) * 16 + plane * 8) = make_uint2(*reinterpret_cast<const uint32_t *>(&h10), *reinterpret_cast<const uint32_t *>(&h11));
-            *reinterpret_cast<uint4 *>(s_a1 + STEM_LBO1 + tid * 16) = make_uint4(0, 0, 0, 0);
-        }
-    }
-    if constexpr (I8) {
-        __syncthreads();
-        const float (*s_dwo)[256][4] = reinterpret_cast<const float (*)[256][4]>(s_a1);
-        const float *s_wp = s_bias2 + 16;
-        const int oy = oy0 + (tid >> 4), ox = ox0 + (tid & 15);
-        if (oy < OH && ox < OW) {
-            const float4 da = *reinterpret_cast<const float4 *>(&s_dwo[0][tid][0]), db = *reinterpret_cast<const float4 *>(&s_dwo[1][tid][0]);
-            const float d[8] = {da.x, da.y, da.z, da.w, db.x, db.y, db.z, db.w};
-            float o[16];
-#pragma unroll
-            for (int j = 0; j < 16; j++) o[j] = s_bias2[j];
-#pragma unroll
-            for (int c = 0; c < 8; c++)
-#pragma unroll
-                for (int j4 = 0; j4 < 4; j4++) {
-                    const float4 wv = *reinterpret_cast<const float4 *>(&s_wp[c * 16 + j4 * 4]);
-                    o[j4 * 4 + 0] = fmaf(d[c], wv.x, o[j4 * 4 + 0]); o[j4 * 4 + 1] = fmaf(d[c], wv.y, o[j4 * 4 + 1]);
-                    o[j4 * 4 + 2] = fmaf(d[c], wv.z, o[j4 * 4 + 2]); o[j4 * 4 + 3] = fmaf(d[c], wv.w, o[j4 * 4 + 3]);
-                }
-            uint32_t pk[4];
-#pragma unroll
-            for (int j4 = 0; j4 < 4; j4++) {
-                uint32_t word = 0;
-#pragma unroll
-                for (int k = 0; k < 4; k++) {
-                    int q = __float2int_rn(__fmul_rn(fmaxf(o[j4 * 4 + k], 0.f), out_inv_scale));
-                    q = max(-127, min(127, q));
-                    word |= (uint32_t)(q & 0xff) << (8 * k);
-                }
-                pk[j4] = word;
-            }
-            *reinterpret_cast<uint4 *>(out + (((size_t)b * OH + oy) * OW + ox) * 16) = make_uint4(pk[0], pk[1], pk[2], pk[3]);
-        }
-    } else {
-    tc::fence_async_smem();
-    __syncthreads();
-    float d1[2][8];
-    {
-        const uint32_t a1 = tc::smem_u32(s_a1), b1 = tc::smem_u32(s_b1);
+        tc::fence_async_smem();
+        __syncthreads();
+        float d1[2][8];
+        {
+            const uint32_t a1 = tc::smem_u32(s_a1), b1 = tc::smem_u32(s_b1);
+#pragma unroll
+            for (int j = 0; j < 2; j++)
+#pragma unroll
+                for (int i = 0; i < 8; i++) d1[j][i] = 0.f;
+            wg::fence();
+#pragma unroll
+            for (int j = 0; j < 2; j++)
+                wg::mma_ss<16>(d1[j], wg::desc(a1 + (uint32_t)(64 * (wgi + 2 * j)) * 16, STEM_LBO1, 128), wg::desc(b1, 256, 128), 0);
+            wg::commit();
+            wg::wait<0>();
+#pragma unroll
+            for (int j = 0; j < 2; j++) wg::fence_regs(d1[j]);
+        }
 #pragma unroll
         for (int j = 0; j < 2; j++)
 #pragma unroll
-            for (int i = 0; i < 8; i++) d1[j][i] = 0.f;
-        wg::fence();
-#pragma unroll
-        for (int j = 0; j < 2; j++)
-            wg::mma_ss<16>(d1[j], wg::desc(a1 + (uint32_t)(64 * (wgi + 2 * j)) * 16, STEM_LBO1, 128), wg::desc(b1, 256, 128), 0);
-        wg::commit();
-        wg::wait<0>();
-#pragma unroll
-        for (int j = 0; j < 2; j++) wg::fence_regs(d1[j]);
-    }
-#pragma unroll
-    for (int j = 0; j < 2; j++)
-#pragma unroll
-        for (int e = 0; e < 2; e++) {
-            const int row = 64 * (wgi + 2 * j) + rl + 8 * e;
-            const int oy = oy0 + (row >> 4), ox = ox0 + (row & 15);
-            if (oy < OH && ox < OW) {
-                __half *dst = reinterpret_cast<__half *>(out) + (((size_t)b * OH + oy) * OW + ox) * 16;
-#pragma unroll
-                for (int i = 0; i < 2; i++) {
-                    const int c = 8 * i + c2;
-                    *reinterpret_cast<__half2 *>(dst + c) = __floats2half2_rn(fmaxf(d1[j][4 * i + 2 * e] + s_bias2[c], 0.f),
-                                                                              fmaxf(d1[j][4 * i + 2 * e + 1] + s_bias2[c + 1], 0.f));
+            for (int e = 0; e < 2; e++) {
+                const int row = 64 * (wgi + 2 * j) + rl + 8 * e;
+                const int oy = oy0 + (row >> 4), ox = ox0 + (row & 15);
+                if (oy < OH && ox < OW) {
+                    __half *dst = reinterpret_cast<__half *>(out) + (((size_t)b * OH + oy) * OW + ox) * 16;
+#pragma unroll
+                    for (int i = 0; i < 2; i++) {
+                        const int c = 8 * i + c2;
+                        *reinterpret_cast<__half2 *>(dst + c) = __floats2half2_rn(fmaxf(d1[j][4 * i + 2 * e] + s_bias2[c], 0.f),
+                                                                                  fmaxf(d1[j][4 * i + 2 * e + 1] + s_bias2[c + 1], 0.f));
+                    }
                 }
             }
         }
diff --git a/retinaface_b200/csrc/tc_conv.cuh b/retinaface_b200/csrc/tc_conv.cuh
--- a/retinaface_b200/csrc/tc_conv.cuh
+++ b/retinaface_b200/csrc/tc_conv.cuh
@@ -73,6 +73,10 @@
     const unsigned sz = valid ? 16u : 0u;
     asm volatile("cp.async.cg.shared.global [%0], [%1], 16, %2;" ::"r"(smem_dst), "l"(gsrc), "r"(sz) : "memory");
 }
+__device__ __forceinline__ void cp_async4(void *smem_dst, const void *gsrc) {
+    asm volatile("cp.async.ca.shared.global [%0], [%1], 4;" ::"r"(tc::smem_u32(smem_dst)), "l"(gsrc) : "memory");
+}
+__device__ __forceinline__ void cp_async_commit() { asm volatile("cp.async.commit_group;" ::: "memory"); }
 __device__ __forceinline__ void cp_async_wait_all() {
     asm volatile("cp.async.commit_group;\n\tcp.async.wait_group 0;" ::: "memory");
 }
diff --git a/retinaface_b200/csrc/tc_dwpw2d.cuh b/retinaface_b200/csrc/tc_dwpw2d.cuh
--- a/retinaface_b200/csrc/tc_dwpw2d.cuh
+++ b/retinaface_b200/csrc/tc_dwpw2d.cuh
@@ -9,6 +9,7 @@
     int N;
     int TH, TW;
     int tiles_x, tiles_y;
+    int run;
     int PH, PW;
     uint32_t lbo_a;
     uint32_t mul_TW, mul_tiles_x, mul_tiles;
@@ -30,7 +31,7 @@
     a.mul_tiles = fast_div_mul((uint32_t)(a.tiles_x * a.tiles_y));
 }
 inline size_t tc_dw2d_smem_bytes(const TcDw2dArgs &a) {
-    return (size_t)a.PH * a.PW * a.C * 2 + (size_t)(a.C / 8) * a.lbo_a + (size_t)a.C * a.N * 2 + 128;
+    return 2 * (size_t)a.PH * a.PW * a.C * 2 + (size_t)(a.C / 8) * a.lbo_a + (size_t)a.C * a.N * 2 + 128;
 }
 
 #ifndef RF_DW2D_OCC
@@ -49,14 +50,16 @@
     const int PH = a.PH, PW = a.PW;
     const uint32_t lbo_a = a.lbo_a;
     const int pix = a.C * 2;
-    unsigned char *sS = smem;
-    unsigned char *sA = smem + (size_t)PH * PW * pix;
+    const uint32_t stage_bytes = (uint32_t)(PH * PW * pix);
+    unsigned char *sA = smem + 2 * (size_t)stage_bytes;
     unsigned char *sB = sA + (size_t)G * lbo_a;
     const int tiles = a.tiles_x * a.tiles_y;
-    const int b = fast_div((int)blockIdx.x, a.mul_tiles), trem = blockIdx.x - b * tiles;
-    const int ty0 = fast_div(trem, a.mul_tiles_x);
-    const int oy0 = ty0 * a.TH, ox0 = (trem - ty0 * a.tiles_x) * a.TW;
-    const int iy0 = oy0 * a.S - 1, ix0 = ox0 * a.S - 1;
+    const int t_end = min((int)blockIdx.x * a.run + a.run, tiles * a.nimg);
+    auto decode = [&](int t, int &b, int &oy0, int &ox0) {
+        b = fast_div(t, a.mul_tiles);
+        const int trem = t - b * tiles, ty0 = fast_div(trem, a.mul_tiles_x);
+        oy0 = ty0 * a.TH; ox0 = (trem - ty0 * a.tiles_x) * a.TW;
+    };
 
     if (tid == 0) {
         tc::mbar_init(&bar_b, 1);
@@ -70,77 +73,88 @@
     for (int i = tid; i < 9 * a.C; i += TC_THREADS) s_dww[i] = dw_weight_f16(a.dw_w[i]);
     if (tid < a.C) s_dwb[tid] = a.dw_b[tid];
     pdl_wait();
-    {
+    const uint32_t sS_s = tc::smem_u32(smem);
+    auto stage = [&](int t, int buf) {
+        int b, oy0, ox0;
+        decode(t, b, oy0, ox0);
+        const int iy0 = oy0 * a.S - 1, ix0 = ox0 * a.S - 1;
         const int per_row = PW << lg;
         const int px_lo = max(0, -ix0), px_hi = min(PW, a.IW - ix0);
         const unsigned px_n = (unsigned)max(px_hi - px_lo, 0);
-        const uint32_t sS_s = tc::smem_u32(sS);
         for (int py = warp; py < PH; py += TC_THREADS / 32) {
             const int iy = iy0 + py;
             const bool rowok = iy >= 0 && iy < a.IH;
             const __half *src_row = a.in + (ptrdiff_t)(((b * a.IH + (rowok ? iy : 0)) * a.IW + ix0) * a.C);
-            const uint32_t dst_row = sS_s + (uint32_t)(py * PW * pix);
+            const uint32_t dst_row = sS_s + (uint32_t)buf * stage_bytes + (uint32_t)(py * PW * pix);
             const __half *zsrc = a.in;
             for (int i = lane; i < per_row; i += 32) {
                 const bool ok = rowok && (unsigned)((i >> lg) - px_lo) < px_n;
                 cp_async16_zfill_s(dst_row + (uint32_t)i * 16u, ok ? src_row + i * 8 : zsrc, ok);
             }
         }
-    }
-    cp_async_wait_all();
-    __syncthreads();
-    const int rows = a.TH * a.TW;
-    auto stencil = [&](auto s_) {
+        cp_async_commit();
+    };
+    auto stencil = [&](auto s_, const unsigned char *sS) {
         constexpr int S = decltype(s_)::value;
-        const int items = (a.TH >> 1) * (a.TW >> 1) << lg;
+        const int items = a.TH * (a.TW >> 1) << lg;
         for (int it = tid; it < items; it += TC_THREADS) {
             const int g = it & (G - 1), rest = it >> lg;
-            const int typ = fast_div(2 * rest, a.mul_TW), ty = 2 * typ, tx = 2 * rest - typ * a.TW;
-            float acc[2][2][8];
+            const int ty = fast_div(2 * rest, a.mul_TW), tx = 2 * rest - ty * a.TW;
+            float acc[1][2][8];
             dw_bias8(acc[0][0], &s_dwb[g * 8]);
 #pragma unroll
-            for (int i = 0; i < 8; i++) { acc[0][1][i] = acc[0][0][i]; acc[1][0][i] = acc[0][0][i]; acc[1][1][i] = acc[0][0][i]; }
-            dw_stencil_block<S, 2, 2>(acc, sS + (ty * S * PW + tx * S) * pix + g * 16, PW * pix, pix, &s_dww[g * 8], a.C);
-            const int r = ty * a.TW + tx;
-            unsigned char *dst = sA + (size_t)g * lbo_a + (size_t)r * 16;
+            for (int i = 0; i < 8; i++) acc[0][1][i] = acc[0][0][i];
+            dw_stencil_block<S, 1, 2>(acc, sS + (ty * S * PW + tx * S) * pix + g * 16, PW * pix, pix, &s_dww[g * 8], a.C);
+            unsigned char *dst = sA + (size_t)g * lbo_a + (size_t)(ty * a.TW + tx) * 16;
             *reinterpret_cast<uint4 *>(dst) = dw_relu_h8(acc[0][0]);
             *reinterpret_cast<uint4 *>(dst + 16) = dw_relu_h8(acc[0][1]);
-            *reinterpret_cast<uint4 *>(dst + a.TW * 16) = dw_relu_h8(acc[1][0]);
-            *reinterpret_cast<uint4 *>(dst + a.TW * 16 + 16) = dw_relu_h8(acc[1][1]);
         }
     };
-    if (a.S == 1) stencil(std::integral_constant<int, 1>{});
-    else stencil(std::integral_constant<int, 2>{});
-    tc::fence_async_smem();
-    __syncthreads();
-    if (64 * (warp >> 2) >= rows) return;
-    tc::mbar_wait(&bar_b, 0);
-    long orow[2];
+    const int rows = a.TH * a.TW;
+    const bool has_gemm = 64 * (warp >> 2) < rows;
+    const int t_begin = (int)blockIdx.x * a.run;
+    stage(t_begin, 0);
+    for (int t = t_begin; t < t_end; t++) {
+        const int buf = (t - t_begin) & 1;
+        cp_async_wait_all();
+        __syncthreads();
+        if (t + 1 < t_end) stage(t + 1, buf ^ 1);
+        const unsigned char *sS = smem + (size_t)buf * stage_bytes;
+        if (a.S == 1) stencil(std::integral_constant<int, 1>{}, sS);
+        else stencil(std::integral_constant<int, 2>{}, sS);
+        tc::fence_async_smem();
+        __syncthreads();
+        if (!has_gemm) continue;
+        tc::mbar_wait(&bar_b, 0);
+        int b, oy0, ox0;
+        decode(t, b, oy0, ox0);
+        long orow[2];
 #pragma unroll
-    for (int e = 0; e < 2; e++) {
-        const int r = tc_frag_row() + 8 * e;
-        const int ty = fast_div(r, a.mul_TW), tx = r - ty * a.TW;
-        const int oy = oy0 + ty, ox = ox0 + tx;
-        orow[e] = (r < rows && oy < a.OH && ox < a.OW) ? (long)((b * a.OH + oy) * a.OW + ox) : -1;
+        for (int e = 0; e < 2; e++) {
+            const int r = tc_frag_row() + 8 * e;
+            const int ty = fast_div(r, a.mul_TW), tx = r - ty * a.TW;
+            const int oy = oy0 + ty, ox = ox0 + tx;
+            orow[e] = (r < rows && oy < a.OH && ox < a.OW) ? (long)((b * a.OH + oy) * a.OW + ox) : -1;
+        }
+        const uint32_t a_addr = tc::smem_u32(sA) + (uint32_t)(64 * (warp >> 2)) * 16u, b_addr = tc::smem_u32(sB);
+        const uint32_t lbo_b = (uint32_t)a.N * 16;
+        const TcOut o{a.out, a.N, a.N, 1, nullptr, 0, 0};
+        wg::for_chunks<(NT < 32 ? NT : 32)>(a.N, [&](auto nc, int n0) {
+            constexpr int NC = decltype(nc)::value;
+            float d[NC / 2];
+            wg::fence();
+            wg::mma_ss<NC>(d, wg::desc(a_addr, lbo_a, 128), wg::desc(b_addr + (uint32_t)n0 * 16u, lbo_b, 128), 0);
+            for (int ks = 1; ks < (a.C >> 4); ks++) {
+                const uint64_t ad = wg::desc(a_addr + (uint32_t)(2 * ks) * lbo_a, lbo_a, 128);
+                const uint64_t bd = wg::desc(b_addr + (uint32_t)(2 * ks) * lbo_b + (uint32_t)n0 * 16u, lbo_b, 128);
+                wg::mma_ss<NC>(d, ad, bd, 1);
+            }
+            wg::commit();
+            wg::wait<0>();
+            wg::fence_regs(d);
+            tc_epilogue<NC>(d, n0, s_bias, o, orow, 0);
+        });
     }
-    const uint32_t a_addr = tc::smem_u32(sA) + (uint32_t)(64 * (warp >> 2)) * 16u, b_addr = tc::smem_u32(sB);
-    const uint32_t lbo_b = (uint32_t)a.N * 16;
-    const TcOut o{a.out, a.N, a.N, 1, nullptr, 0, 0};
-    wg::for_chunks<(NT < 32 ? NT : 32)>(a.N, [&](auto nc, int n0) {
-        constexpr int NC = decltype(nc)::value;
-        float d[NC / 2];
-        wg::fence();
-        wg::mma_ss<NC>(d, wg::desc(a_addr, lbo_a, 128), wg::desc(b_addr + (uint32_t)n0 * 16u, lbo_b, 128), 0);
-        for (int ks = 1; ks < (a.C >> 4); ks++) {
-            const uint64_t ad = wg::desc(a_addr + (uint32_t)(2 * ks) * lbo_a, lbo_a, 128);
-            const uint64_t bd = wg::desc(b_addr + (uint32_t)(2 * ks) * lbo_b + (uint32_t)n0 * 16u, lbo_b, 128);
-            wg::mma_ss<NC>(d, ad, bd, 1);
-        }
-        wg::commit();
-        wg::wait<0>();
-        wg::fence_regs(d);
-        tc_epilogue<NC>(d, n0, s_bias, o, orow, 0);
-    });
 }
 
 }
```
